# arpg/Kangaroo

Hardware: AMD Instinct MI355X
Metric: kinectfusion_frames_per_sec_640x480_to_512cubed_tsdf (higher is better)
Workload: dtype f32

## Files before the change

### include/kfx_debug.h

```cpp
#ifndef KFX_DEBUG_H
#define KFX_DEBUG_H

#include "kfx.h"

#ifdef __cplusplus
extern "C" {
#endif

int kfx_debug_rmw(const kfx_volume* vol, int variant, kfx_stream stream);

int kfx_debug_div_uniform_check(float b, unsigned long long* d_out, kfx_stream stream);

int kfx_debug_div_core_check(unsigned seed, int per_divisor, unsigned long long* d_out, kfx_stream stream);
int kfx_debug_sqrt_core_check(unsigned long long* d_out, kfx_stream stream);
int kfx_debug_wave_xor_check(unsigned seed, unsigned long long* d_out, kfx_stream stream);

int kfx_debug_summary_export(kfx_sdf_summary* s, float tol, float vref, int fine_shift, void* R_out, void* C_out, int dims_out[12],
                             kfx_stream stream);

int kfx_debug_summary_conditional_builds(kfx_sdf_summary* s, int out[2], kfx_stream stream);

int kfx_debug_summary_top_levels(kfx_sdf_summary* s, int fine_shift, void* top_out, int dims_out[12], unsigned long long* launches_out,
                                 kfx_stream stream);

int kfx_debug_fuse_keep(const kfx_sdf_summary* s, int out[3], unsigned char* kept, int n_rows);

#ifdef __cplusplus
}
#endif
#endif
```

### kangaroo_amd/csrc/debug.hip

```cpp
#include "kfx_device.h"
#include "sampling.h"
#include "../../include/kfx_debug.h"

namespace kfx {

__global__ __launch_bounds__(256) void k_rmw_linear(float4* __restrict__ base, size_t n4)
{
    const size_t stride = (size_t)gridDim.x * blockDim.x;
    for (size_t i = (size_t)blockIdx.x * blockDim.x + threadIdx.x; i < n4; i += stride) {
        float4 c = base[i];
        c.y += 1.0f;
        c.w += 1.0f;
        base[i] = c;
    }
}

template <int ZC>
__global__ __launch_bounds__(256) void k_rmw_brick(unsigned char* vptr, size_t pitch, size_t img_pitch, int X, int Y, int Z)
{
    const int tid = threadIdx.x, lane = tid & 63, wv = tid >> 6;
    const int x0 = (blockIdx.x * 32 + (lane & 31)) * 2;
    const int y = blockIdx.y * 8 + wv * 2 + (lane >> 5);
    const int zbeg = blockIdx.z * ZC, zend = min(zbeg + ZC, Z);
    if (x0 >= X || y >= Y) return;
    unsigned char* cell = vptr + (size_t)zbeg * img_pitch + (size_t)y * pitch + (size_t)x0 * 8;
    for (int z = zbeg; z < zend; ++z, cell += img_pitch) {
        float4 c = *reinterpret_cast<const float4*>(cell);
        c.y += 1.0f;
        c.w += 1.0f;
        *reinterpret_cast<float4*>(cell) = c;
    }
}

template <int ZC>
__global__ __launch_bounds__(256) void k_rmw_rows(unsigned char* vptr, size_t pitch, size_t img_pitch, int X, int Y, int Z)
{
    const int lane = threadIdx.x & 63, wv = threadIdx.x >> 6;
    const int x0 = (blockIdx.x * 64 + lane) * 2;
    const int y = blockIdx.y * 4 + wv;
    const int zbeg = blockIdx.z * ZC, zend = min(zbeg + ZC, Z);
    if (x0 >= X || y >= Y) return;
    unsigned char* cell = vptr + (size_t)zbeg * img_pitch + (size_t)y * pitch + (size_t)x0 * 8;
    for (int z = zbeg; z < zend; ++z, cell += img_pitch) {
        float4 c = *reinterpret_cast<const float4*>(cell);
        c.y += 1.0f;
        c.w += 1.0f;
        *reinterpret_cast<float4*>(cell) = c;
    }
}

__global__ __launch_bounds__(256) void k_rmw_column(unsigned char* vptr, size_t pitch, size_t img_pitch, int X, int Y, int Z)
{
    const int lane = threadIdx.x & 63, wv = threadIdx.x >> 6;
    const int x0 = (blockIdx.x * 64 + lane) * 2;
    const int y = blockIdx.y * 4 + wv;
    if (x0 >= X || y >= Y) return;
    unsigned char* cell = vptr + (size_t)y * pitch + (size_t)x0 * 8;
    for (int z = 0; z < Z; ++z, cell += img_pitch) {
        float4 c = *reinterpret_cast<const float4*>(cell);
        c.y += 1.0f;
        c.w += 1.0f;
        *reinterpret_cast<float4*>(cell) = c;
    }
}

typedef float v4f_dbg __attribute__((ext_vector_type(4)));
template <int WX, int WY, int ZC, bool NT>
__global__ __launch_bounds__(256) void k_rmw_gen(unsigned char* vptr, size_t pitch, size_t img_pitch, int X, int Y, int Z)
{
    const int lane = threadIdx.x & 63, wv = threadIdx.x >> 6;
    const int x0 = ((blockIdx.x * WX + (wv % WX)) * 64 + lane) * 2;
    const int y = blockIdx.y * WY + (wv / WX);
    const int zbeg = blockIdx.z * ZC, zend = min(zbeg + ZC, Z);
    if (x0 >= X || y >= Y) return;
    unsigned char* cell = vptr + (size_t)zbeg * img_pitch + (size_t)y * pitch + (size_t)x0 * 8;
    for (int z = zbeg; z < zend; ++z, cell += img_pitch) {
        v4f_dbg c;
        if constexpr (NT) c = __builtin_nontemporal_load(reinterpret_cast<const v4f_dbg*>(cell));
        else c = *reinterpret_cast<const v4f_dbg*>(cell);
        c.y += 1.0f;
        c.w += 1.0f;
        if constexpr (NT) __builtin_nontemporal_store(c, reinterpret_cast<v4f_dbg*>(cell));
        else *reinterpret_cast<v4f_dbg*>(cell) = c;
// ... 154 lines not shown
    GEN(12, 1, 4, 16, false)
    GEN(13, 1, 4, 16, true)
    GEN(14, 4, 1, 16, true)
    GEN(15, 1, 4, 1, false)
    GEN(16, 1, 4, 64, false)
    GEN(17, 4, 1, 4, false)
    GEN(18, 2, 2, 16, true)
#undef GEN
    default: return set_error(KFX_E_RANGE, "kfx_debug_rmw: variant");
    }
    return check_launch("kfx_debug_rmw");
}

static int last_published(const kfx_sdf_summary* s)
{
    if (!s->h_skippable || !s->builds) return -2;
    const uint64_t v = __atomic_load_n(s->h_skippable + summary_ring_index(s->builds - 1), __ATOMIC_ACQUIRE);
    return summary_ring_slot_stamp(v) == summary_ring_stamp(s->builds - 1) ? summary_ring_slot_count(v) : -1;
}

extern "C" int kfx_debug_summary_export(kfx_sdf_summary* s, float tol, float vref, int fine_shift, void* R_out, void* C_out, int dims_out[12],
                                        kfx_stream stream)
{
    if (!s || !dims_out) return set_error(KFX_E_NULL, "kfx_debug_summary_export: null argument");
    if (fine_shift < 3 || fine_shift > 5) return set_error(KFX_E_RANGE, "kfx_debug_summary_export: fine_shift in [3, 5]");
    ClassView cv;
    summary_class_layout(s, fine_shift, cv);
    dims_out[0] = s->nbx; dims_out[1] = s->nby; dims_out[2] = s->nbz;
    dims_out[3] = cv.fine.first; dims_out[4] = cv.fine.rw; dims_out[5] = cv.fine.ny;
    dims_out[6] = cv.coarse.first; dims_out[7] = cv.coarse.rw; dims_out[8] = cv.coarse.ny;
    dims_out[9] = cv.words; dims_out[10] = s->n_coarse; dims_out[11] = last_published(s);
    const size_t n = (size_t)s->nbx * s->nby * s->nbz;
    hipStream_t st = (hipStream_t)stream;
    if (R_out && hipMemcpyAsync(R_out, s->R, n * sizeof(float4), hipMemcpyDeviceToDevice, st) != hipSuccess) return set_error(KFX_E_RANGE, "kfx_debug_summary_export: copy");
    if (C_out) {
        if (int e = summary_classes_prepare(s, tol, vref, fine_shift, st)) return e;
        if (hipMemcpyAsync(C_out, s->C, (size_t)cv.words * sizeof(unsigned), hipMemcpyDeviceToDevice, st) != hipSuccess || hipStreamSynchronize(st) != hipSuccess)
            return set_error(KFX_E_RANGE, "kfx_debug_summary_export: copy");
        dims_out[11] = last_published(s);
    }
    return 0;
}

extern "C" int kfx_debug_summary_conditional_builds(kfx_sdf_summary* s, int out[2], kfx_stream stream)
{
    if (!s || !out) return set_error(KFX_E_NULL, "kfx_debug_summary_conditional_builds: null argument");
    hipStream_t st = (hipStream_t)stream;
    if (hipMemcpyAsync(out, s->d_count + 3, 2 * sizeof(int), hipMemcpyDeviceToHost, st) != hipSuccess || hipStreamSynchronize(st) != hipSuccess)
        return set_error(KFX_E_RANGE, "kfx_debug_summary_conditional_builds: copy");
    return 0;
}

extern "C" int kfx_debug_summary_top_levels(kfx_sdf_summary* s, int fine_shift, void* top_out, int dims_out[12], unsigned long long* launches_out, kfx_stream stream)
{
    if (!s || !dims_out) return set_error(KFX_E_NULL, "kfx_debug_summary_top_levels: null argument");
    if (fine_shift < 3 || fine_shift > 5) return set_error(KFX_E_RANGE, "kfx_debug_summary_top_levels: fine_shift in [3, 5]");
    ClassView cv;
    summary_class_layout(s, fine_shift, cv);
    cv.nx5 = ceil_div(s->w, 32); cv.nz5 = ceil_div(s->d, 32);
    ClassLevel l6, l7;
    int w6, w7;
    summary_top_layout(cv, l6, l7, w6, w7);
    const int nx6 = (cv.nx5 + 1) >> 1, nz6 = (cv.nz5 + 1) >> 1;
    dims_out[0] = l6.first - cv.words; dims_out[1] = l6.rw; dims_out[2] = l6.ny; dims_out[3] = nx6; dims_out[4] = nz6; dims_out[5] = w6;
    dims_out[6] = l7.first - cv.words; dims_out[7] = l7.rw; dims_out[8] = l7.ny; dims_out[9] = (nx6 + 1) >> 1; dims_out[10] = (nz6 + 1) >> 1; dims_out[11] = w7;
    if (launches_out) *launches_out = s->launches;
    if (top_out) {
        if (s->c_shift != fine_shift) return set_error(KFX_E_RANGE, "kfx_debug_summary_top_levels: the tables held were built for another fine level");
        hipStream_t st = (hipStream_t)stream;
        if (hipMemcpyAsync(top_out, s->C + cv.words, (size_t)(w6 + w7) * sizeof(unsigned), hipMemcpyDeviceToDevice, st) != hipSuccess || hipStreamSynchronize(st) != hipSuccess)
            return set_error(KFX_E_RANGE, "kfx_debug_summary_top_levels: copy");
    }
    return 0;
}

extern "C" int kfx_debug_fuse_keep(const kfx_sdf_summary* s, int out[3], unsigned char* kept, int n_rows)
{
    if (!s || !out) return set_error(KFX_E_NULL, "kfx_debug_fuse_keep: null argument");
    out[0] = s->keep_stride; out[1] = s->keep_row0; out[2] = s->keep_rows;
    for (int r = 0; kept && r < n_rows; ++r)
        kept[r] = (r >= s->keep_row0 && r < s->keep_row0 + s->keep_rows && keep_row(r, s->keep_stride)) ? 1 : 0;
    return 0;
}
```

### kangaroo_amd/csrc/frame.hip

```cpp
#include <cmath>
#include <cstdlib>
#include <new>

#include "kfx_device.h"
#include "frame_host.h"
#include "sensor_host.h"
#include "shift_host.h"

struct kfx_frame {
    kfx_frame_config cfg;
    kfx_sdf_summary* summary;
    int track;
    long long frames;
    kfx::EventRing ring;
    unsigned mask;
    kfx_image texels;
    kfx_depth_input* input;
};

using namespace kfx;

extern "C" int kfx_frame_create(kfx_frame** out, const kfx_frame_config* cfg)
{
    if (!out || !cfg) return set_error(KFX_E_NULL, "kfx_frame_create: null argument");
    *out = nullptr;
    if (!cfg->vol.ptr) return set_error(KFX_E_NULL, "kfx_frame_create: null volume");
    if (int e = check_frame_views(cfg->raw, cfg->filtered, cfg->vbo, cfg->normals, cfg->ray_depth, cfg->ray_norm, cfg->ray_img, "kfx_frame_create")) return e;
    if (cfg->timing_slots < 0 || cfg->timing_slots > (1 << 20)) return set_error(KFX_E_RANGE, "kfx_frame_create: timing_slots");
    kfx_frame* f = new (std::nothrow) kfx_frame;
    if (!f) return set_error(KFX_E_RANGE, "kfx_frame_create: out of memory");
    f->cfg = *cfg;
    f->summary = nullptr;
    f->track = 0;
    f->frames = 0;
    f->mask = KFX_FRAME_EVENTS_ALL;
    f->input = nullptr;
    f->texels = texel_image_alloc(cfg->filtered.w, cfg->filtered.h);
    if (int e = ring_create(f->ring, 4, cfg->timing_slots, -1, "kfx_frame_create")) {
        texel_image_free(f->texels);
        delete f;
        return e;
    }
    *out = f;
    return 0;
}

extern "C" int kfx_frame_destroy(kfx_frame* f)
{
    if (!f) return 0;
    if (f->summary) kfx_sdf_summary_destroy(f->summary);
    ring_destroy(f->ring);
    texel_image_free(f->texels);
    delete f;
    return 0;
}

extern "C" int kfx_frame_set_timing(kfx_frame* f, unsigned mask)
{
    if (!f) return set_error(KFX_E_NULL, "kfx_frame_set_timing: null frame");
    if (mask > KFX_FRAME_EVENTS_ALL) return set_error(KFX_E_RANGE, "kfx_frame_set_timing: mask");
    f->mask = mask;
    return 0;
}

extern "C" int kfx_frame_get_track(const kfx_frame* f) { return f ? f->track : set_error(KFX_E_NULL, "kfx_frame_get_track: null frame"); }
extern "C" kfx_sdf_summary* kfx_frame_summary(kfx_frame* f) { return f ? f->summary : nullptr; }
extern "C" long long kfx_frame_count(const kfx_frame* f) { return f ? f->frames : 0; }

kfx_volume* kfx::frame_volume(kfx_frame* f) { return &f->cfg.vol; }
kfx_sdf_summary* kfx::frame_tracked_summary(kfx_frame* f) { return f->track ? f->summary : nullptr; }

extern "C" int kfx_frame_set_track(kfx_frame* f, int on, kfx_stream stream)
{
    if (!f) return set_error(KFX_E_NULL, "kfx_frame_set_track: null frame");
    if (!on) {
        f->track = 0;
        return 0;
    }
    if (!f->summary)
        if (int e = kfx_sdf_summary_create(&f->summary, &f->cfg.vol)) return e;
    if (!f->track)
        if (int e = kfx_sdf_summary_rebuild(f->summary, stream)) return e;
    f->track = 1;
    return 0;
}

extern "C" int kfx_frame_set_input(kfx_frame* f, kfx_depth_input* in)
{
    if (!f) return set_error(KFX_E_NULL, "kfx_frame_set_input: null frame");
    if (in && !depth_input_matches(in, f->cfg.filtered.w, f->cfg.filtered.h)) return set_error(KFX_E_SHAPE, "kfx_frame_set_input: the ring's image size differs from the frame's");
    f->input = in;
    return 0;
}

extern "C" int kfx_frame_reset(kfx_frame* f, kfx_stream stream)
{
    if (!f) return set_error(KFX_E_NULL, "kfx_frame_reset: null frame");
    const float nan = __builtin_nanf("");
    if (f->track) return kfx_sdf_reset_tracked(&f->cfg.vol, f->summary, nan, stream);
    return kfx_sdf_reset(&f->cfg.vol, nan, stream);
}

extern "C" int kfx_frame_step(kfx_frame* f, const kfx_image* raw, const float T_wc[12], const float* T_cw, unsigned parts, kfx_stream stream)
{
    if (!f || !T_wc) return set_error(KFX_E_NULL, "kfx_frame_step: null argument");
    if (parts == 0) parts = KFX_FRAME_PREPROCESS | KFX_FRAME_FUSE | KFX_FRAME_RAYCAST;
    const kfx_frame_config& c = f->cfg;
    const kfx_image* src = raw ? raw : &c.raw;
    float inv[12];
    if (!T_cw) {
        se3_inverse(T_wc, inv);
        T_cw = inv;
    }
    kfx_depth_input* const sensor = (!raw && (parts & KFX_FRAME_PREPROCESS)) ? f->input : nullptr;
    if (sensor)
        if (int e0 = depth_input_wait(sensor, stream)) return e0;
    ring_begin(f->ring, f->frames, f->mask);
    int e = 0;
    const auto record = [&](int k) {
        const hipError_t he = ring_record(f->ring, f->frames, k, (hipStream_t)stream);
        if (he != hipSuccess && !e) e = set_error((int)he, "kfx_frame_step: hipEventRecord");
    };
    record(0);
    const kfx_image* tex = ((parts & KFX_FRAME_PREPROCESS) && (parts & KFX_FRAME_FUSE) && f->texels.ptr) ? &f->texels : nullptr;
    if (!e && (parts & KFX_FRAME_PREPROCESS)) {
        if (sensor) e = depth_input_consume(sensor, &c.filtered, &c.raw, c.bilateral_gs, c.bilateral_gr, c.bilateral_size, c.bilateral_minval, stream);
        else e = kfx_bilateral_f32(&c.filtered, src, c.bilateral_gs, c.bilateral_gr, c.bilateral_size, c.bilateral_minval, 1, stream);
        if (!e) e = depth_to_vbo_normals_texels(&c.vbo, &c.normals, &c.filtered, c.K, 1.0f, tex, stream);
    }
    record(1);
    if (!e && (parts & KFX_FRAME_FUSE))
        e = sdf_fuse_texels(&c.vol, f->track ? f->summary : nullptr, &c.filtered, &c.normals, tex, T_cw, c.K, c.trunc_dist, c.max_w, c.mincostheta, c.fuse_flags, stream);
    record(2);
    if (!e && (parts & KFX_FRAME_RAYCAST)) {
        if (f->track) e = kfx_raycast_sdf_tracked(&c.ray_depth, &c.ray_norm, &c.ray_img, &c.vol, f->summary, T_wc, c.K, c.near, c.far, c.trunc_dist, 1, stream);
        else e = kfx_raycast_sdf(&c.ray_depth, &c.ray_norm, &c.ray_img, &c.vol, T_wc, c.K, c.near, c.far, c.trunc_dist, 1, stream);
    }
    record(3);
    f->frames += 1;
    return e;
}

static void frame_spans(const EventRing& r, long long fr, float* o, hipError_t& he)
{
    o[0] = ring_span(r, fr, 0, 1, he);
    o[1] = ring_span(r, fr, 1, 2, he);
    o[2] = ring_span(r, fr, 2, 3, he);
    o[3] = ring_span(r, fr, 0, 3, he);
    o[4] = ring_period(r, fr, he);
}

extern "C" int kfx_frame_timings(kfx_frame* f, long long first_frame, int n_frames, float* ms)
{
    if (!f || !ms) return set_error(KFX_E_NULL, "kfx_frame_timings: null argument");
    return ring_timings(f->ring, f->frames, first_frame, n_frames, KFX_FRAME_TIMING_FIELDS, ms, frame_spans, "kfx_frame_timings");
}
```

### kangaroo_amd/csrc/frame_host.h

```cpp
#pragma once

#include <new>

#include "kfx_device.h"
#include "host_args.h"

namespace kfx {

inline int check_frame_views(const kfx_image& raw, const kfx_image& filtered, const kfx_image& vbo, const kfx_image& normals, const kfx_image& ray_depth,
                             const kfx_image& ray_norm, const kfx_image& ray_img, const char* what)
{
    const struct { const kfx_image* im; size_t elem; } views[7] = {{&raw, 4}, {&filtered, 4}, {&vbo, 16}, {&normals, 16}, {&ray_depth, 4}, {&ray_norm, 16}, {&ray_img, 4}};
    for (const auto& v : views) {
        if (!v.im->ptr) return fail_rule(what, KFX_E_SHAPE, "image views");
        if (int e = check_image(v.im, v.elem, 1, 1, what)) return e;
    }
    if (filtered.w != raw.w || filtered.h != raw.h || vbo.w != raw.w || vbo.h != raw.h || normals.w != raw.w || normals.h != raw.h)
        return fail_rule(what, KFX_E_SHAPE, "the preprocess images differ in size");
    return 0;
}

inline void se3_inverse(const float T_wc[12], float out[12])
{
    for (int i = 0; i < 3; ++i) {
        double t = 0.0;
        for (int j = 0; j < 3; ++j) {
            out[i * 4 + j] = T_wc[j * 4 + i];
            t += (double)T_wc[j * 4 + i] * (double)T_wc[j * 4 + 3];
        }
        out[i * 4 + 3] = (float)-t;
    }
}

inline kfx_image texel_image_alloc(size_t w, size_t h)
{
    const TexLayout tl = tex_layout(w, h);
    void* buf = nullptr;
    if (tl.tpitch < (1u << 24) && hipMalloc(&buf, tl.bytes) == hipSuccess) return kfx_image{tl.tpitch, buf, w, h};
    (void)hipGetLastError();
    return kfx_image{0, nullptr, 0, 0};
}
inline void texel_image_free(kfx_image& t)
{
    if (t.ptr) { (void)hipFree(t.ptr); (void)hipGetLastError(); }
    t = kfx_image{0, nullptr, 0, 0};
}

struct EventRing {
    int n = 0, slots = 0;
    int side = -1;
    hipEvent_t* ev = nullptr;
    long long* frame = nullptr;
    unsigned char* want = nullptr;
    unsigned char* mask = nullptr;
};

inline void ring_destroy(EventRing& r)
{
    if (r.ev)
        for (int i = 0; i < r.slots * r.n; ++i) if (r.ev[i]) (void)hipEventDestroy(r.ev[i]);
    delete[] r.ev; delete[] r.frame; delete[] r.want; delete[] r.mask;
    r = EventRing{};
}

inline int ring_create(EventRing& r, int n, int slots, int side, const char* what)
{
    r = EventRing{};
    if (!slots) return 0;
    r.n = n; r.slots = slots; r.side = side;
    r.ev = new (std::nothrow) hipEvent_t[(size_t)slots * n]();
    r.frame = new (std::nothrow) long long[slots];
    r.want = new (std::nothrow) unsigned char[slots]();
    r.mask = new (std::nothrow) unsigned char[slots]();
    int e = (r.ev && r.frame && r.want && r.mask) ? 0 : fail_rule(what, KFX_E_RANGE, "out of memory");
    for (int i = 0; !e && i < slots; ++i) r.frame[i] = -1;
    for (int i = 0; !e && i < slots * n; ++i) {
        const hipError_t he = hipEventCreate(&r.ev[i]);
        if (he != hipSuccess) { (void)hipGetLastError(); r.ev[i] = nullptr; e = fail_rule(what, (int)he, "hipEventCreate"); }
    }
    if (e) ring_destroy(r);
    return e;
}

inline void ring_begin(EventRing& r, long long frame, unsigned mask)
{
    if (!r.slots) return;
    const int slot = (int)(frame % r.slots);
    r.frame[slot] = mask ? frame : -1;
    r.want[slot] = (unsigned char)mask;
    r.mask[slot] = 0;
}

inline hipError_t ring_record(EventRing& r, long long frame, int k, hipStream_t stream)
{
    if (!r.slots) return hipSuccess;
    const int slot = (int)(frame % r.slots);
    if (r.frame[slot] != frame || !(r.want[slot] & (1u << k))) return hipSuccess;
    const hipError_t he = hipEventRecord(r.ev[(size_t)slot * r.n + k], stream);
    if (he == hipSuccess) r.mask[slot] |= (unsigned char)(1u << k);
    else (void)hipGetLastError();
    return he;
}

inline unsigned ring_recorded(const EventRing& r, long long frame)
{
    return frame >= 0 && r.frame[frame % r.slots] == frame ? (unsigned)r.mask[frame % r.slots] : 0u;
}
inline hipEvent_t ring_event(const EventRing& r, long long frame, int k) { return r.ev[(size_t)(frame % r.slots) * r.n + k]; }
inline int first_event(unsigned m) { return m ? __builtin_ctz(m) : -1; }
inline int last_event(unsigned m) { return m ? 31 - __builtin_clz(m) : -1; }

inline hipError_t ring_wait(const EventRing& r, long long first, long long last)
{
    hipEvent_t wait_for = nullptr;
    const int b = first_event(ring_recorded(r, last));
    if (b >= 0 && (ring_recorded(r, last + 1) & (1u << b))) wait_for = ring_event(r, last + 1, b);
    for (long long fr = last; !wait_for && fr >= first; --fr)
        if (ring_recorded(r, fr)) wait_for = ring_event(r, fr, last_event(ring_recorded(r, fr)));
    hipError_t he = wait_for ? hipEventSynchronize(wait_for) : hipSuccess;
    for (long long fr = last; r.side >= 0 && he == hipSuccess && fr >= first; --fr)
        if (ring_recorded(r, fr) & (1u << r.side)) he = hipEventSynchronize(ring_event(r, fr, r.side));
    return he;
}
// ... 39 lines not shown
```

### kangaroo_amd/csrc/fuse.hip

```cpp
#include <cmath>
#include <cstring>

#include <sys/syscall.h>
#include <unistd.h>

#include <hip/hip_fp16.h>

#include <type_traits>

#include "kfx_device.h"
#include "../../include/kfx_slab_color.h"
#include "host_args.h"

#ifndef KFX_FUSE_STAGE_DMA
#define KFX_FUSE_STAGE_DMA 1
#endif

namespace kfx {

constexpr int FUSE_ZC = 16;
constexpr int FUSE_ROWS = 4;
constexpr int TB_X = 64, TB_Y = 8;

struct FuseParams {
    unsigned char* vptr;
    size_t vpitch, vimg_pitch;
    int X, Y, Z;
    int zoff;
    float w1, h1, d1;
    V3 bmin, size;
    Pose T;
    Intr K;
    ImgView depth;
    ImgView norm;
    float dwb, dhb;
    float trunc, max_w, mincos;
    unsigned dpitch, npitch;
    int exact_shared;
    int z_rev, keep_stride, keep_row0;
    float4* sum_R;
    int sum_nbx, sum_nby;
    int sum_bx0, sum_by0, sum_bz0;
    int sum_w, sum_h, sum_d;
    float sum_lo_ok, sum_hi_ok;
    int* sum_dirty;
    int zoff_local;
    int xcd_swizzle;
    int fuse_cull;
    const unsigned char* tex;
    unsigned tpitch;
    const float* bmax;
    unsigned bw8;
    float inv_w1, inv_h1;
    int pos_div;
};

__device__ __forceinline__ float voxel_pos(float bmin, float size, int i, float n1, float inv_n1, int pos_div)
{
    const float a = size * (float)i;
    return bmin + (pos_div ? div_uniform(a, n1, inv_n1) : a / n1);
}

__device__ __forceinline__ float slice_z(const FuseParams& p, int z) { return p.bmin.z + p.size.z * (float)(z + p.zoff) / p.d1; }

__device__ __forceinline__ int xcd_rotated_brick(const FuseParams& p, int bzi)
{
    return p.xcd_swizzle ? (int)((blockIdx.x + (bzi >> (p.xcd_swizzle - 1))) % gridDim.x) : (int)blockIdx.x;
}

struct TileRect {
    int x0, y0, w, h;
    __device__ __forceinline__ bool fits(int cap) const { return w > 1 && h > 1 && w * h <= cap; }
};
__device__ __forceinline__ TileRect tile_rect(float lo_u, float hi_u, float lo_v, float hi_v, int img_w, int img_h)
{
    const float fx0 = fmaxf(floorf(lo_u) - 1.f, 0.f), fx1 = fminf(floorf(hi_u) + 2.f, (float)(img_w - 1));
    const float fy0 = fmaxf(floorf(lo_v) - 1.f, 0.f), fy1 = fminf(floorf(hi_v) + 2.f, (float)(img_h - 1));
    TileRect r;
    r.x0 = (int)fx0; r.y0 = (int)fy0;
    r.w = (int)fx1 - r.x0 + 1; r.h = (int)fy1 - r.y0 + 1;
    return r;
}
__device__ __forceinline__ bool misses_band(float lo_u, float hi_u, float lo_v, float hi_v, float wb, float hb)
{
    return hi_u < 2.0f || !(lo_u < wb) || hi_v < 2.0f || !(lo_v < hb);
}

__device__ __forceinline__ float far_depth(float dmax) { return dmax + fabsf(dmax) * 1e-5f; }
__device__ __forceinline__ bool brick_occluded(float dmax, float zmin, const FuseParams& p)
{
    return far_depth(dmax) - zmin < -(p.trunc / p.mincos) * 1.001f;
}

struct Obs {
    float val, w;
    bool ok;
};

struct Corners { float4 c00, c01, c10, c11; };
__device__ __forceinline__ Corners tile_corners(const float4* t, int tw)
{
    Corners c;
    c.c00 = t[0]; c.c01 = t[1]; c.c10 = t[tw]; c.c11 = t[tw + 1];
    return c;
}
struct CornersDx { float4 c00, d0, c10, d1; };
__device__ __forceinline__ CornersDx tile_corners_dx(const float4* t, int tw)
{
    return CornersDx{t[0], t[1], t[2 * tw], t[2 * tw + 1]};
}

typedef float v4f __attribute__((ext_vector_type(4)));

__device__ __forceinline__ float lerp_f(float a, float b, float t) { return __builtin_fmaf(t, b - a, a); }

template <bool FAST>
struct CamXY {
    float ax, ay, az;
    __device__ __forceinline__ void init(const FuseParams& p, float px, float py)
    {
        if constexpr (FAST) {
            ax = __builtin_fmaf(p.T.m[0], px, __builtin_fmaf(p.T.m[1], py, p.T.m[3]));
            ay = __builtin_fmaf(p.T.m[4], px, __builtin_fmaf(p.T.m[5], py, p.T.m[7]));
            az = __builtin_fmaf(p.T.m[8], px, __builtin_fmaf(p.T.m[9], py, p.T.m[11]));
        } else {
            ax = p.T.m[0] * px + p.T.m[1] * py;
            ay = p.T.m[4] * px + p.T.m[5] * py;
            az = p.T.m[8] * px + p.T.m[9] * py;
        }
    }
    __device__ __forceinline__ V3 at(const FuseParams& p, float pz) const
    {
        if constexpr (FAST)
            return v3(__builtin_fmaf(p.T.m[2], pz, ax), __builtin_fmaf(p.T.m[6], pz, ay), __builtin_fmaf(p.T.m[10], pz, az));
        else
            return v3(ax + p.T.m[2] * pz + p.T.m[3], ay + p.T.m[6] * pz + p.T.m[7], az + p.T.m[10] * pz + p.T.m[11]);
    }
};

template <bool FAST>
__device__ __forceinline__ void project(const FuseParams& p, const V3 Pc, float& pu, float& pv, float& iz)
{
    if constexpr (FAST) {
        iz = __builtin_amdgcn_rcpf(Pc.z);
        pu = __builtin_fmaf(p.K.fu * Pc.x, iz, p.K.u0);
        pv = __builtin_fmaf(p.K.fv * Pc.y, iz, p.K.v0);
    } else {
        iz = 0.f;
        pu = p.K.u0 + p.K.fu * Pc.x / Pc.z;
        pv = p.K.v0 + p.K.fv * Pc.y / Pc.z;
    }
}

__device__ __forceinline__ bool in_bounds(const FuseParams& p, float pu, float pv)
{
    return 2.0f <= pu && pu < p.dwb && 2.0f <= pv && pv < p.dhb;
}

__device__ __forceinline__ Corners fetch_global64(const FuseParams& p, int ix, int iy)
{
    const float* dbl = row<float>(p.depth, (size_t)iy) + ix;
    const float* dtl = row<float>(p.depth, (size_t)iy + 1) + ix;
    const float4* nbl = row<float4>(p.norm, (size_t)iy) + ix;
    const float4* ntl = row<float4>(p.norm, (size_t)iy + 1) + ix;
    const float4 n00 = nbl[0], n01 = nbl[1], n10 = ntl[0], n11 = ntl[1];
    Corners c;
    c.c00 = make_float4(n00.x, n00.y, n00.z, dbl[0]);
    c.c01 = make_float4(n01.x, n01.y, n01.z, dbl[1]);
    c.c10 = make_float4(n10.x, n10.y, n10.z, dtl[0]);
    c.c11 = make_float4(n11.x, n11.y, n11.z, dtl[1]);
    return c;
}

struct __attribute__((packed, aligned(4))) P2 { float a, b; };
__device__ __forceinline__ Corners fetch_global32(const FuseParams& p, int ix, int iy)
{
    const unsigned od = __umul24((unsigned)iy, p.dpitch) + (unsigned)ix * 4u;
    const unsigned on = __umul24((unsigned)iy, p.npitch) + (unsigned)ix * 16u;
    const P2 db = *reinterpret_cast<const P2*>(p.depth.ptr + od);
    const P2 dt = *reinterpret_cast<const P2*>(p.depth.ptr + p.dpitch + od);
    const float4* nb = reinterpret_cast<const float4*>(p.norm.ptr + on);
    const float4* nt = reinterpret_cast<const float4*>(p.norm.ptr + p.npitch + on);
    const float4 n00 = nb[0], n01 = nb[1], n10 = nt[0], n11 = nt[1];
    Corners c;
    c.c00 = make_float4(n00.x, n00.y, n00.z, db.a);
    c.c01 = make_float4(n01.x, n01.y, n01.z, db.b);
    c.c10 = make_float4(n10.x, n10.y, n10.z, dt.a);
    c.c11 = make_float4(n11.x, n11.y, n11.z, dt.b);
    return c;
}

template <bool FAST>
__device__ __forceinline__ Obs finish(const FuseParams& p, const V3 Pc, float iz, float fx, float fy, const Corners& c)
{
    Obs o;
    o.ok = false;
    o.val = 0.f;
    o.w = 0.f;
    float md, costheta, w;
    if constexpr (FAST) {
        md = lerp_f(lerp_f(c.c00.w, c.c01.w, fx), lerp_f(c.c10.w, c.c11.w, fx), fy);
        const float nx = lerp_f(lerp_f(c.c00.x, c.c01.x, fx), lerp_f(c.c10.x, c.c11.x, fx), fy);
        const float ny = lerp_f(lerp_f(c.c00.y, c.c01.y, fx), lerp_f(c.c10.y, c.c11.y, fx), fy);
        const float nz = lerp_f(lerp_f(c.c00.z, c.c01.z, fx), lerp_f(c.c10.z, c.c11.z, fx), fy);
        const float dotn = __builtin_fmaf(nz, Pc.z, __builtin_fmaf(ny, Pc.y, nx * Pc.x));
        const float len2 = __builtin_fmaf(Pc.z, Pc.z, __builtin_fmaf(Pc.y, Pc.y, Pc.x * Pc.x));
        costheta = -dotn * __builtin_amdgcn_rsqf(len2);
        w = costheta * iz;
    } else {
        md = lerp(lerp(c.c00.w, c.c01.w, fx), lerp(c.c10.w, c.c11.w, fx), fy);
        V3 mdn;
        mdn.x = lerp(lerp(c.c00.x, c.c01.x, fx), lerp(c.c10.x, c.c11.x, fx), fy);
        mdn.y = lerp(lerp(c.c00.y, c.c01.y, fx), lerp(c.c10.y, c.c11.y, fx), fy);
        mdn.z = lerp(lerp(c.c00.z, c.c01.z, fx), lerp(c.c10.z, c.c11.z, fx), fy);
        costheta = dot(mdn, Pc) / -length(Pc);
        w = costheta * 1.0f / Pc.z;
    }
    const float sd = costheta * (md - Pc.z);
    o.ok = ((int)!(sd <= -p.trunc) & (int)isfinite(md) & (int)isfinite(w) & (int)(costheta > p.mincos)) != 0;
    if constexpr (FAST) o.val = __builtin_amdgcn_fmed3f(sd, -p.trunc, p.trunc);
    else o.val = clampf(sd, -p.trunc, p.trunc);
    o.w = w;
    return o;
}

__device__ __forceinline__ Obs finish_shared(const FuseParams& p, const V3 Pc, float yz, float fx, float fy, const Corners& c)
{
    Obs o;
    const float md = lerp(lerp(c.c00.w, c.c01.w, fx), lerp(c.c10.w, c.c11.w, fx), fy);
    V3 mdn;
    mdn.x = lerp(lerp(c.c00.x, c.c01.x, fx), lerp(c.c10.x, c.c11.x, fx), fy);
    mdn.y = lerp(lerp(c.c00.y, c.c01.y, fx), lerp(c.c10.y, c.c11.y, fx), fy);
    mdn.z = lerp(lerp(c.c00.z, c.c01.z, fx), lerp(c.c10.z, c.c11.z, fx), fy);
    const float nlen = -sqrt_core(dot(Pc, Pc));
    const float costheta = div_core(dot(mdn, Pc), nlen, rcp_nr(nlen));
// ... 131 lines not shown
    o.w = 0.f;
    float pu, pv, iz;
    project<FAST>(p, Pc, pu, pv, iz);
    if (in_bounds(p, pu, pv)) {
        const float fix = floorf(pu), fiy = floorf(pv);
        const Corners c = TEX ? fetch_texels(p, (int)fix, (int)fiy) : (OFF32 ? fetch_global32(p, (int)fix, (int)fiy) : fetch_global64(p, (int)fix, (int)fiy));
        o = finish<FAST>(p, Pc, iz, pu - fix, pv - fiy, c);
    }
    return o;
}

template <int VEC, bool FAST, bool OFF32, typename CELL>
__global__ __launch_bounds__(256) void k_sdf_fuse(const FuseParams p)
{
    __shared__ float s_pz[FUSE_ZC];
    const int lane = threadIdx.x & 63, wv = threadIdx.x >> 6;
    const int x0 = (blockIdx.x * 64 + lane) * VEC;
    const int y = blockIdx.y * FUSE_ROWS + wv;
    const int zbeg = blockIdx.z * FUSE_ZC;
    const int zend = min(zbeg + FUSE_ZC, p.Z);
    if (threadIdx.x < FUSE_ZC)
        s_pz[threadIdx.x] = slice_z(p, zbeg + (int)threadIdx.x);
    __syncthreads();
    if (x0 >= p.X || y >= p.Y) return;

    const float py = p.bmin.y + p.size.y * (float)y / p.h1;
    CamXY<FAST> cam[VEC];
#pragma unroll
    for (int v = 0; v < VEC; ++v) cam[v].init(p, p.bmin.x + p.size.x * (float)(x0 + v) / p.w1, py);

    unsigned char* cell = p.vptr + (size_t)zbeg * p.vimg_pitch + (size_t)y * p.vpitch + (size_t)x0 * CELL::BYTES;
    for (int z = zbeg; z < zend; ++z, cell += p.vimg_pitch) {
        const float pz = s_pz[z - zbeg];
        Obs o[VEC];
#pragma unroll
        for (int v = 0; v < VEC; ++v) o[v] = observe<FAST, OFF32>(p, cam[v].at(p, pz));
        if constexpr (VEC == 2) {
            if (o[0].ok || o[1].ok) {
                float4 c = CELL::ld2(cell);
                accumulate_pair<FAST, CELL>(o[0], o[1], p.max_w, c);
                CELL::st2(cell, c);
            }
        } else {
            if (o[0].ok) {
                float2 c = CELL::ld1(cell);
                accumulate<FAST, CELL>(o[0], p.max_w, c.x, c.y);
                CELL::st1(cell, c);
            }
        }
    }
}

template <bool FAST, int ZU, typename CELL, int LX = 32, int WY = 4, int ZC = FUSE_ZC, bool TRACK = false, bool DXT = false, int NW = 4>
__global__ __launch_bounds__(64 * NW, (FAST && ZU == 2) ? 8 : (!FAST ? 6 : 1)) void k_sdf_fuse_tiled(const FuseParams p_arg, const int cap_px)
{
    static_assert(!DXT || (!FAST && !TRACK), "the difference tile belongs to the bit-exact, untracked kernels");
    FuseParams p = p_arg;
    constexpr bool PARK = !(FAST && TRACK);
    if constexpr (PARK) {
        p.T.m[2] = in_vgpr(p.T.m[2]); p.T.m[6] = in_vgpr(p.T.m[6]); p.T.m[10] = in_vgpr(p.T.m[10]);
        if constexpr (!FAST) { p.T.m[3] = in_vgpr(p.T.m[3]); p.T.m[7] = in_vgpr(p.T.m[7]); p.T.m[11] = in_vgpr(p.T.m[11]); }
        p.K.fu = in_vgpr(p.K.fu); p.K.fv = in_vgpr(p.K.fv); p.K.u0 = in_vgpr(p.K.u0); p.K.v0 = in_vgpr(p.K.v0);
    }
    constexpr int NT = 64 * NW, RW = 64 / LX, WZ = NW / WY, ZW = ZC / WZ, BY = RW * WY;
    static_assert(LX * RW == 64 && WY * WZ == NW && ZW * WZ == ZC && ZW % ZU == 0, "brick geometry");
    static_assert(NW == 4 || (NW == 8 && !TRACK), "the summary epilogue is written for four waves");
    constexpr int NG = ZW / 8, NXB = LX / 4, NZB = ZC / 8;
    static_assert(!TRACK || (BY == 8 && ZW % 8 == 0 && NG <= 2 && 8 % ZU == 0), "summary bricks are 8 x 8 x 8");
    __shared__ float s_part[TRACK ? 4 * 2 * 8 * 3 : 1];
    extern __shared__ __attribute__((aligned(16))) float4 s_tile[];
    __shared__ float s_pz[ZC];
    __shared__ float s_dmax[NW], s_cmin[NW];
    __shared__ float4 s_tz[ZC];
    const int tid = threadIdx.x, lane = tid & 63, wv = __builtin_amdgcn_readfirstlane(tid >> 6);
    const int bzi = (TRACK && p.z_rev) ? (int)(gridDim.z - 1 - blockIdx.z) : (int)blockIdx.z;
    const int bxi = xcd_rotated_brick(p, bzi);
    const int x0 = (bxi * LX + (lane & (LX - 1))) * 2;
    const int y = blockIdx.y * BY + (wv % WY) * RW + lane / LX;
    const int zbeg = bzi * ZC;
    const bool keep = TRACK && keep_row(p.keep_row0 + (int)blockIdx.y, p.keep_stride);
    const int zend = min(zbeg + ZC, p.Z);
    const int wz0 = zbeg + (wv / WY) * ZW, wz1 = min(wz0 + ZW, zend);
    const bool live = x0 < p.X && y < p.Y;
    if (tid < ZC) {
        const float pz = slice_z(p, zbeg + tid);
        s_pz[tid] = pz;
        if constexpr (!FAST) s_tz[tid] = make_float4(pz, p.T.m[2] * pz, p.T.m[6] * pz, p.T.m[10] * pz);
    }
    __syncthreads();

    const float py = voxel_pos(p.bmin.y, p.size.y, y, p.h1, p.inv_h1, p.pos_div);
    CamXY<FAST> cam[2];
#pragma unroll
    for (int v = 0; v < 2; ++v) cam[v].init(p, voxel_pos(p.bmin.x, p.size.x, x0 + v, p.w1, p.inv_w1, p.pos_div), py);

    float umin, umax, vmin, vmax, zmin, cmax = 0.f;
    bool any_bad;
    {
        const int c = lane & 7;
        const int xb0 = bxi * LX * 2, yb0 = (int)blockIdx.y * BY;
        const int xc = (c & 1) ? min(xb0 + LX * 2, p.X) - 1 : xb0;
        const int yc = (c & 2) ? min(yb0 + BY, p.Y) - 1 : yb0;
        const float pzc = s_pz[(c & 4) ? (zend - 1 - zbeg) : 0];
        CamXY<FAST> cc;
        cc.init(p, voxel_pos(p.bmin.x, p.size.x, xc, p.w1, p.inv_w1, p.pos_div), voxel_pos(p.bmin.y, p.size.y, yc, p.h1, p.inv_h1, p.pos_div));
        const V3 Pc = cc.at(p, pzc);
        float pu, pv, iz;
        project<FAST>(p, Pc, pu, pv, iz);
        const bool bad = !(Pc.z > 0.f) || !(fabsf(pu) < 1e9f) || !(fabsf(pv) < 1e9f);
        const FMin fmin2;
        const FMax fmax2;
        const auto uni = [](float x) { return __uint_as_float((unsigned)__builtin_amdgcn_readfirstlane((int)__float_as_uint(x))); };
        umin = uni(wave8_combine(pu, fmin2)); umax = uni(wave8_combine(pu, fmax2));
        vmin = uni(wave8_combine(pv, fmin2)); vmax = uni(wave8_combine(pv, fmax2));
        zmin = uni(wave8_combine(Pc.z, fmin2));
        if constexpr (!FAST) cmax = uni(wave8_combine(fmaxf(fmaxf(fabsf(Pc.x), fabsf(Pc.y)), Pc.z), fmax2));
        any_bad = __ballot(bad) != 0ull;
    }

    bool use_tile = false;
    TileRect tile = {0, 0, 0, 0};
    if (!any_bad) {
        if (misses_band(umin, umax, vmin, vmax, p.dwb, p.dhb)) return;
        tile = tile_rect(umin, umax, vmin, vmax, p.depth.w, p.depth.h);
        use_tile = tile.fits(cap_px);
        if constexpr (DXT) use_tile = use_tile && p.exact_shared && zmin >= 0x1p-20f && cmax <= 0x1p20f;
    }
    const int tx0 = tile.x0, ty0 = tile.y0, tw = tile.w, th = tile.h;
    const bool whole = !TRACK || ((bxi + 1) * LX * 2 <= p.X && ((int)blockIdx.y + 1) * BY <= p.Y);
    const bool interior = __builtin_amdgcn_readfirstlane((int)(use_tile && whole && umin >= 2.01f && umax < p.dwb - 0.01f && vmin >= 2.01f && vmax < p.dhb - 0.01f)) != 0;
    float dmax = -__builtin_inff();
    constexpr bool DMA = KFX_FUSE_STAGE_DMA && !DXT;
    if constexpr (DMA) {
        if (use_tile) {
            const unsigned lane16 = (unsigned)lane * 16u;
            const unsigned lds0 = (unsigned)(size_t)(__attribute__((address_space(3))) char*)(char*)s_tile;
            const int tail = tw & 63;
            const unsigned long long mask_tail = tail ? ((1ull << tail) - 1ull) : ~0ull;
            const int chunks = (tw + 63) >> 6;
            for (int r = wv; r < th; r += NW) {
                const unsigned char* rowp = p.tex + ((size_t)(ty0 + r) * p.tpitch + (size_t)tx0 * 16u);
                unsigned dst = lds0 + (unsigned)(r * tw) * 16u;
#pragma unroll 1
                for (int c = 0; c < chunks; ++c, rowp += 1024, dst += 1024u) {
                    const unsigned long long m = (c + 1 == chunks) ? mask_tail : ~0ull;
                    unsigned long long keep_exec;
                    unsigned keep_m0;
                    asm volatile("s_mov_b64 %0, exec\n\t"
                                 "s_mov_b32 %1, m0\n\t"
                                 "s_mov_b64 exec, %2\n\t"
                                 "s_mov_b32 m0, %3\n\t"
                                 "s_nop 0\n\t"
                                 "global_load_lds_dwordx4 %4, %5\n\t"
                                 "s_mov_b32 m0, %1\n\t"
                                 "s_mov_b64 exec, %0"
                                 : "=&s"(keep_exec), "=&s"(keep_m0)
                                 : "s"(m), "s"(dst), "v"(lane16), "s"(rowp)
                                 : "memory");
                }
            }
            {
                const int bx0 = tx0 >> 3, nbx = ((tx0 + tw - 1) >> 3) - bx0 + 1, by0 = ty0 >> 2, nb = nbx * (((ty0 + th - 1) >> 2) - by0 + 1);
                const float inv_nbx = 1.0f / (float)nbx;
                for (int i = tid; i < nb; i += NT) {
                    const int br = (int)(((float)i + 0.5f) * inv_nbx);
                    dmax = fmaxf(dmax, p.bmax[(size_t)(by0 + br) * p.bw8 + (size_t)(bx0 + i - br * nbx)]);
                }
                block_put(s_dmax, wv, dmax, FMax{});
            }
            asm volatile("s_waitcnt vmcnt(0)" ::: "memory");
        }
    }
    if (!DMA && use_tile) {
        if constexpr (FAST) {
            const int ntex = tw * th;
            const float inv_tw = 1.0f / (float)tw;
            constexpr int SU = 4;
            for (int t0 = tid; t0 < ntex; t0 += NT * SU) {
                float4 n[SU];
                float d[SU];
#pragma unroll
                for (int k = 0; k < SU; ++k) {
                    const int t = t0 + k * NT;
                    n[k] = make_float4(0.f, 0.f, 0.f, 0.f);
                    d[k] = -__builtin_inff();
                    if (t < ntex) {
                        const int r = (int)(((float)t + 0.5f) * inv_tw);
                        const int c = t - r * tw;
                        const unsigned y = (unsigned)(ty0 + r), x = (unsigned)(tx0 + c);
                        n[k] = *reinterpret_cast<const float4*>(p.norm.ptr + (__umul24(y, p.npitch) + x * 16u));
                        d[k] = *reinterpret_cast<const float*>(p.depth.ptr + (__umul24(y, p.dpitch) + x * 4u));
                    }
                }
#pragma unroll
                for (int k = 0; k < SU; ++k) {
                    const int t = t0 + k * NT;
                    if (t < ntex) {
                        s_tile[t] = make_float4(n[k].x, n[k].y, n[k].z, d[k]);
                        dmax = fmaxf(dmax, d[k]);
                    }
                }
            }
        } else {
            for (int r = wv; r < th; r += NW) {
                const float* drow = row<float>(p.depth, (size_t)(ty0 + r)) + tx0;
                const float4* nrow = row<float4>(p.norm, (size_t)(ty0 + r)) + tx0;
                for (int c = lane; c < tw; c += 64) {
                    const float4 n = nrow[c];
                    const float d = drow[c];
                    s_tile[(r * tw + c) * (DXT ? 2 : 1)] = make_float4(n.x, n.y, n.z, d);
                    dmax = fmaxf(dmax, d);
                }
            }
// ... 123 lines not shown
                const float fix = floorf(pu), fiy = floorf(pv);
                const int ix = (int)fix, iy = (int)fiy;
                const unsigned rx = (unsigned)(ix - tx0), ry = (unsigned)(iy - ty0);
                Corners c;
                if (use_tile && rx < (unsigned)(tw - 1) && ry < (unsigned)(th - 1)) {
                    c = tile_corners(s_tile + (ry * (unsigned)tw + rx), tw);
                } else {
                    c = DMA ? fetch_texels(p, ix, iy) : fetch_global32(p, ix, iy);
                }
                o = finish<FAST>(p, Pc, iz, pu - fix, pv - fiy, c);
            }
            return o;
        };

        unsigned char* cell = p.vptr + (size_t)wz0 * p.vimg_pitch + (size_t)y * p.vpitch + (size_t)x0 * CELL::BYTES;

        if constexpr (!FAST) {
            if (use_tile && p.exact_shared && zmin >= 0x1p-20f && cmax <= 0x1p20f) {
                const int cxmax = in_vgpr(tw - 2), cymax = in_vgpr(th - 2), tx0v = in_vgpr(tx0), ty0v = in_vgpr(ty0);
                auto observe_pair = [&](auto interior_c, int z, Obs (&o)[2]) -> bool {
                    constexpr bool INTERIOR = decltype(interior_c)::value;
                    const float4 tz = s_tz[z - zbeg];
                    bool stray = false;
    #pragma unroll
                    for (int v = 0; v < 2; ++v) {
                        const V3 Pc = v3(cam[v].ax + tz.y + p.T.m[3], cam[v].ay + tz.z + p.T.m[7], cam[v].az + tz.w + p.T.m[11]);
                        const float yz = rcp_nr(Pc.z);
                        const float pu = p.K.u0 + div_core(p.K.fu * Pc.x, Pc.z, yz);
                        const float pv = p.K.v0 + div_core(p.K.fv * Pc.y, Pc.z, yz);
                        const float fix = floorf(pu), fiy = floorf(pv);
                        const int rx = (int)fix - tx0v, ry = (int)fiy - ty0v;
                        const auto sample = [&](int at) {
                            if constexpr (DXT) return finish_shared(p, Pc, yz, pu - fix, pv - fiy, tile_corners_dx(s_tile + 2 * at, tw));
                            else return finish_shared(p, Pc, yz, pu - fix, pv - fiy, tile_corners(s_tile + at, tw));
                        };
                        if constexpr (INTERIOR) {
                            o[v] = sample(ry * tw + rx);
                        } else {
                            const bool inb = upd && in_bounds(p, pu, pv), inside = cell_inside(rx, ry, cxmax, cymax);
                            o[v] = sample(cell_clamped(rx, ry, cxmax, cymax, tw));
                            stray |= gate_sample(o[v], inb, inside);
                        }
                    }
                    if constexpr (!INTERIOR) {
                        if (__builtin_expect(__ballot(stray) != 0ull, 0)) {
                            o[0] = observe<false, true, DMA>(p, cam[0].at(p, tz.x));
                            o[1] = observe<false, true, DMA>(p, cam[1].at(p, tz.x));
                            o[0].ok = o[0].ok && upd; o[1].ok = o[1].ok && upd;
                        }
                    }
                    return ((int)o[0].ok | (int)o[1].ok) != 0;
                };
                auto shared_loop = [&](auto interior_c) {
                for (int z = wz0; z < wz1; z += ZU, cell += (size_t)ZU * p.vimg_pitch) {
                    next_group(z);
                    Obs o[ZU][2];
                    bool any[ZU];
    #pragma unroll
                    for (int k = 0; k < ZU; ++k) {
                        any[k] = false;
                        if (z + k < wz1) {
                            any[k] = observe_pair(interior_c, z + k, o[k]);
                            note_pair(o[k][0].ok, o[k][1].ok);
                        }
                    }
                    float4 c[ZU];
                    load_cells(c, any, cell);
    #pragma unroll
                    for (int k = 0; k < ZU; ++k)
                        if (any[k]) {
                            accumulate_pair<false, CELL>(o[k][0], o[k][1], p.max_w, c[k]);
                            CELL::st2(cell + (size_t)k * p.vimg_pitch, c[k]);
                            note_vals(c[k]);
                        }
                }
                };
                if (interior) shared_loop(std::true_type{});
                else shared_loop(std::false_type{});
                flush();
                return;
            }
        }
        if (use_tile) {
            const int cxmax = PARK ? in_vgpr(tw - 2) : tw - 2, cymax = PARK ? in_vgpr(th - 2) : th - 2, tx0v = PARK ? in_vgpr(tx0) : tx0,
                      ty0v = PARK ? in_vgpr(ty0) : ty0;
            auto tiled_loop = [&](auto interior_c) {
            constexpr bool INTERIOR = decltype(interior_c)::value;
            for (int z = wz0; z < wz1; z += ZU, cell += (size_t)ZU * p.vimg_pitch) {
                next_group(z);
                Obs o[ZU][2];
                bool any[ZU];
                bool stray = false;
    #pragma unroll
                for (int k = 0; k < ZU; ++k) {
                    any[k] = false;
                    if (z + k < wz1) {
                        const float pz = s_pz[z + k - zbeg];
    #pragma unroll
                        for (int v = 0; v < 2; ++v) {
                            const V3 Pc = cam[v].at(p, pz);
                            float pu, pv, iz;
                            project<FAST>(p, Pc, pu, pv, iz);
                            const float fix = floorf(pu), fiy = floorf(pv);
                            const int rx = (int)fix - tx0v, ry = (int)fiy - ty0v;
                            if constexpr (INTERIOR) {
                                o[k][v] = finish<FAST>(p, Pc, iz, pu - fix, pv - fiy, tile_corners(s_tile + (ry * tw + rx), tw));
                            } else {
                                const bool inb = upd && in_bounds(p, pu, pv), inside = cell_inside(rx, ry, cxmax, cymax);
                                o[k][v] = finish<FAST>(p, Pc, iz, pu - fix, pv - fiy, tile_corners(s_tile + cell_clamped(rx, ry, cxmax, cymax, tw), tw));
                                stray |= gate_sample(o[k][v], inb, inside);
                            }
                        }
                        any[k] = ((int)o[k][0].ok | (int)o[k][1].ok) != 0;
                    }
                }
                if constexpr (!INTERIOR) {
                if (__builtin_expect(__ballot(stray) != 0ull, 0)) {
    #pragma unroll
                    for (int k = 0; k < ZU; ++k)
                        if (z + k < wz1) {
                            const float pz = s_pz[z + k - zbeg];
                            o[k][0] = observe<FAST, true, DMA>(p, cam[0].at(p, pz));
                            o[k][1] = observe<FAST, true, DMA>(p, cam[1].at(p, pz));
                            o[k][0].ok = o[k][0].ok && upd; o[k][1].ok = o[k][1].ok && upd;
                            any[k] = o[k][0].ok || o[k][1].ok;
                        }
                }
                }
    #pragma unroll
                for (int k = 0; k < ZU; ++k)
                    if (z + k < wz1) note_pair(o[k][0].ok, o[k][1].ok);
                float4 c[ZU];
                load_cells(c, any, cell);
    #pragma unroll
                for (int k = 0; k < ZU; ++k)
                    if (any[k]) {
                        if (o[k][0].ok) accumulate<FAST, CELL>(o[k][0], p.max_w, c[k].x, c[k].y);
                        if (o[k][1].ok) accumulate<FAST, CELL>(o[k][1], p.max_w, c[k].z, c[k].w);
                        CELL::st2(cell + (size_t)k * p.vimg_pitch, c[k]);
                        note_vals(c[k]);
                    }
            }
            };
            if (interior) tiled_loop(std::true_type{});
            else tiled_loop(std::false_type{});
            flush();
            return;
        }
        for (int z = wz0; z < wz1; z += ZU, cell += (size_t)ZU * p.vimg_pitch) {
            next_group(z);
            Obs o[ZU][2];
            bool any[ZU];
    #pragma unroll
            for (int k = 0; k < ZU; ++k) {
                any[k] = false;
                if (z + k < wz1) {
                    const float pz = s_pz[z + k - zbeg];
                    o[k][0] = observe_tile(0, pz);
                    o[k][1] = observe_tile(1, pz);
                    o[k][0].ok = o[k][0].ok && upd; o[k][1].ok = o[k][1].ok && upd;
                    any[k] = o[k][0].ok || o[k][1].ok;
                    note_pair(o[k][0].ok, o[k][1].ok);
                }
            }
            float4 c[ZU];
            load_cells(c, any, cell);
    #pragma unroll
// ... 408 lines not shown
        }
        block_put(s_dmax, wv, dmax, FMax{});
    }
    __syncthreads();
    if (use_tile && p.mincos > 0.f && p.trunc > 0.f && brick_occluded(block_get<4>(s_dmax, FMax{}), zmin, p)) return;
    if constexpr (!TRACK) {
        if (!live) return;
    }
    const bool upd = !TRACK || live;
    ColorTrack trk;
    trk.reset(0);

    unsigned char* cell = p.vptr + (size_t)zbeg * p.vimg_pitch + (size_t)y * p.vpitch + (size_t)x0 * 8;
    unsigned char* ccell = q.cptr + (size_t)zbeg * q.cimg_pitch + (size_t)y * q.cpitch + (size_t)x0 * 4;
    const int cxmax = tw - 2, cymax = th - 2, gxmax = cw - 2, gymax = chh - 2;
    for (int z = zbeg; z < zend; ++z, cell += p.vimg_pitch, ccell += q.cimg_pitch) {
        if constexpr (TRACK) trk.next_group(s_part, wv, lane, zend - zbeg, z - zbeg);
        const float pz = s_pz[z - zbeg];
        Obs o[2];
        float grey[2];
        bool stray = !use_tile;
        if (use_tile) {
#pragma unroll
            for (int v = 0; v < 2; ++v) {
                const V3 Pc = cam[v].at(p, pz), Pi = ccam[v].at(q, pz);
                float pu, pv, iz, qu, qv;
                project<FAST>(p, Pc, pu, pv, iz);
                project_color<FAST>(q, Pi, qu, qv);
                const bool inb = upd && in_bounds(p, pu, pv) && in_bounds_color(q, qu, qv);
                const float fix = floorf(pu), fiy = floorf(pv), gix = floorf(qu), giy = floorf(qv);
                const int rx = (int)fix - tx0, ry = (int)fiy - ty0, gx = (int)gix - cx0, gy = (int)giy - cy0;
                const bool inside = cell_inside(rx, ry, cxmax, cymax) && cell_inside(gx, gy, gxmax, gymax);
                o[v] = finish<FAST>(p, Pc, iz, pu - fix, pv - fiy, tile_corners(s_tile + cell_clamped(rx, ry, cxmax, cymax, tw), tw));
                stray |= gate_sample(o[v], inb, inside);
                const unsigned* g = s_rgb + cell_clamped(gx, gy, gxmax, gymax, cw);
                const Rgb4 texels{g[0], g[1], g[cw], g[cw + 1]};
                if constexpr (FAST) {
                    grey[v] = grey_bilinear<true>(texels, qu - gix, qv - giy);
                } else {
                    grey[v] = 0.f;
                    if (o[v].ok) grey[v] = grey_bilinear<false>(texels, qu - gix, qv - giy);
                }
            }
        }
        if (__builtin_expect(__ballot(stray) != 0ull, 0)) {
#pragma unroll
            for (int v = 0; v < 2; ++v) {
                o[v] = observe_color_global<FAST>(p, q, cam[v].at(p, pz), ccam[v].at(q, pz), grey[v]);
                o[v].ok = o[v].ok && upd;
            }
        }
        if constexpr (TRACK) trk.note_pair(o[0].ok, o[1].ok);
        if (o[0].ok || o[1].ok) {
            float4 c = CellF32::ld2(cell);
            const v2f k = __builtin_nontemporal_load(reinterpret_cast<const v2f*>(ccell));
            float k0 = k.x, k1 = k.y;
            if (o[0].ok) k0 = color_mean<FAST>(o[0].w, grey[0], k0, c.y);
            if (o[1].ok) k1 = color_mean<FAST>(o[1].w, grey[1], k1, c.w);
            accumulate_pair<FAST, CellF32>(o[0], o[1], p.max_w, c);
            CellF32::st2(cell, c);
            v2f kk;
            kk.x = k0; kk.y = k1;
            __builtin_nontemporal_store(kk, reinterpret_cast<v2f*>(ccell));
            if constexpr (TRACK) trk.note_vals(c);
        }
    }
    if constexpr (TRACK) {
        trk.flush(s_part, wv, lane, zend - zbeg);
        __syncthreads();
        color_track_epilogue(p, s_part, tid, bxi, zbeg);
    }
}

__global__ __launch_bounds__(256) void k_fill_f32(float* __restrict__ base, size_t n, float v)
{
    for (size_t i = (size_t)blockIdx.x * 256 + threadIdx.x; i < n; i += (size_t)gridDim.x * 256) base[i] = v;
}

}

using namespace kfx;

__global__ __launch_bounds__(256) void k_pack_texels(const ImgView depth, const ImgView norm, unsigned char* __restrict__ tex, const size_t tpitch,
                                                     float* __restrict__ bmax, const unsigned bw8)
{
    __shared__ float s_max[PIX_H][8];
    int u, v, lane, wv;
    pixel_xy(u, v, lane, wv);
    float d = -__builtin_inff();
    if (u < depth.w && v < depth.h) {
        d = row<float>(depth, (size_t)v)[u];
        texel_put(tex, tpitch, u, v, row<float4>(norm, (size_t)v)[u], d);
    }
    texel_block_max(bmax, bw8, lane, wv, d, s_max);
}

struct TexScratch {
    static constexpr int N = 4;
    struct Entry { void* buf; size_t bytes; hipStream_t stream; int device; unsigned long used; };
    Entry e[N] = {};
    unsigned long tick = 0;
    bool main_thread = false;
    ~TexScratch()
    {
        if (main_thread) return;
        for (Entry& x : e)
            if (x.buf) { (void)hipFree(x.buf); (void)hipGetLastError(); }
    }
    void* get(size_t bytes, hipStream_t stream)
    {
        int dev = 0;
        if (hipGetDevice(&dev) != hipSuccess) { (void)hipGetLastError(); return nullptr; }
        Entry* hit = nullptr;
        Entry* lru = &e[0];
        for (Entry& x : e) {
            if (x.buf && x.stream == stream && x.device == dev) { hit = &x; break; }
            if (!x.buf) { if (lru->buf) lru = &x; } else if (lru->buf && x.used < lru->used) lru = &x;
        }
        if (!hit) {
            hit = lru;
            if (hit->buf) {
                (void)hipFree(hit->buf); (void)hipGetLastError();
                hit->buf = nullptr; hit->bytes = 0;
            }
            hit->stream = stream; hit->device = dev;
        }
        if (hit->bytes < bytes) {
            if (hit->buf) { (void)hipFree(hit->buf); (void)hipGetLastError(); hit->buf = nullptr; hit->bytes = 0; }
            if (hipMalloc(&hit->buf, bytes) != hipSuccess) { (void)hipGetLastError(); hit->buf = nullptr; return nullptr; }
            hit->bytes = bytes;
        }
        hit->used = ++tick;
        return hit->buf;
    }
};
static void* tex_scratch(size_t bytes, hipStream_t stream)
{
    thread_local TexScratch pool;
    static const long main_tid = (long)getpid();
    pool.main_thread = (long)syscall(SYS_gettid) == main_tid;
    return pool.get(bytes, stream);
}

static VolView vol_view(const kfx_volume* vol)
{
    VolView v;
    v.ptr = (unsigned char*)vol->ptr;
    v.pitch = vol->pitch;
    v.img_pitch = vol->img_pitch;
    v.w = (int)vol->w;
    v.h = (int)vol->h;
    v.d = (int)vol->d;
    v.bmin = V3{vol->boxmin[0], vol->boxmin[1], vol->boxmin[2]};
    v.bmax = V3{vol->boxmax[0], vol->boxmax[1], vol->boxmax[2]};
    return v;
}

static bool pos_div_verified(int axis, float size, int dim)
{
    struct Memo { float size; int dim; bool ok; };
    static thread_local Memo memo[2] = {{0.0f, 0, false}, {0.0f, 0, false}};
    Memo& m = memo[axis];
    if (m.dim == dim && memcmp(&m.size, &size, sizeof(float)) == 0) return m.ok;
    const float n1 = (float)(dim - 1), inv = 1.0f / n1;
    bool ok = div_uniform_safe_host(size) && div_uniform_safe_host(size * n1);
    for (int i = 0; ok && i < dim; ++i) {
        const float a = size * (float)i;
        const float q0 = a * inv;
        const float q = fmaf(fmaf(-n1, q0, a), inv, q0), d = a / n1;
// ... 21 lines not shown
    p.Z = full ? (int)vol->d : (int)(vol->d / 8) * 8;
    if (!full && (flags & KFX_FUSE_SLAB_EXTENT) && slab) {
        const size_t zlim = (slab->full_d / 8) * 8;
        const size_t z_end = slab->z_offset + vol->d < zlim ? slab->z_offset + vol->d : zlim;
        p.Z = z_end > slab->z_offset ? (int)(z_end - slab->z_offset) : 0;
    }
    p.w1 = (float)(vol->w - 1);
    p.h1 = (float)(vol->h - 1);
    p.d1 = (float)(vol->d - 1);
    p.bmin = V3{vol->boxmin[0], vol->boxmin[1], vol->boxmin[2]};
    p.size = V3{vol->boxmax[0] - vol->boxmin[0], vol->boxmax[1] - vol->boxmin[1], vol->boxmax[2] - vol->boxmin[2]};
    if (slab) {
        if (slab->full_d < 2 || slab->z_offset + vol->d > slab->full_d) return set_error(KFX_E_SHAPE, "SdfFuse: slab outside the full volume");
        p.d1 = (float)(slab->full_d - 1);
        p.zoff = (int)slab->z_offset;
        p.bmin.z = slab->full_zmin;
        p.size.z = slab->full_zmax - slab->full_zmin;
    }
    for (int i = 0; i < 12; ++i) p.T.m[i] = T_cw[i];
    p.K = Intr{K[0], K[1], K[2], K[3]};
    p.depth = ImgView{(const unsigned char*)depth->ptr, depth->pitch, (int)depth->w, (int)depth->h};
    p.norm = ImgView{(const unsigned char*)norm->ptr, norm->pitch, (int)norm->w, (int)norm->h};
    p.dwb = (float)depth->w - 2.0f;
    p.dhb = (float)depth->h - 2.0f;
    p.trunc = trunc_dist;
    p.max_w = max_w;
    p.mincos = mincostheta;
    *small_images = depth->pitch * depth->h < (1ull << 31) && norm->pitch * norm->h < (1ull << 31) &&
                    depth->pitch < (1u << 24) && norm->pitch < (1u << 24) && depth->h < (1u << 24);
    p.dpitch = *small_images ? (unsigned)depth->pitch : 0u;
    p.npitch = *small_images ? (unsigned)norm->pitch : 0u;
    p.inv_w1 = 1.0f / p.w1;
    p.inv_h1 = 1.0f / p.h1;
    static const int pos_div_env = env_int("KFX_FUSE_POS_DIV", 1);
    p.pos_div = (pos_div_env && vol->w >= 2 && vol->h >= 2 && pos_div_verified(0, p.size.x, (int)vol->w) && pos_div_verified(1, p.size.y, (int)vol->h)) ? 1 : 0;
    static const int swizzle_env = env_int("KFX_FUSE_XCD_SWIZZLE", 1, 0, 8);
    p.xcd_swizzle = swizzle_env;
    static const int cull_env = env_int("KFX_FUSE_CULL", 1);
    p.fuse_cull = cull_env;
    static const int shared_env = env_int("KFX_FUSE_EXACT_SHARED", 1);
    const float afu = fabsf(p.K.fu), afv = fabsf(p.K.fv);
    p.exact_shared = shared_env && afu >= 0x1p-20f && afu <= 0x1p20f && afv >= 0x1p-20f && afv <= 0x1p20f &&
                     mincostheta >= 0x1p-20f && mincostheta < __builtin_inff() && trunc_dist > 0.f && trunc_dist < __builtin_inff();
    return 0;
}

static float px_per_voxel(const FuseParams& p, const Pose& T, const Intr& K, int z0, int z1)
{
    const float cx = p.bmin.x + 0.5f * p.size.x, cy = p.bmin.y + 0.5f * p.size.y;
    const float cz = p.bmin.z + p.size.z * (0.5f * (float)(z0 + z1 - 1) + (float)p.zoff) / p.d1;
    const float Zc = T.m[8] * cx + T.m[9] * cy + T.m[10] * cz + T.m[11];
    if (!(Zc > 0.f)) return 0.f;
    const float voxel = fmaxf(p.size.x / p.w1, p.size.y / p.h1);
    return fmaxf(fabsf(K.fu), fabsf(K.fv)) * voxel / Zc;
}

static int tile_cap(const FuseParams& p, const Pose& T, const Intr& K, int z0, int z1, bool small_ok = false)
{
    const float r = px_per_voxel(p, T, K, z0, z1);
    static const float r_small = env_float("KFX_FUSE_R_SMALL", 0.85f);
    if (small_ok && !(r > r_small)) return 1216;
    if (!(r > 1.3f)) return 1536;
    const float want = 1536.f * (r / 1.05f) * (r / 1.05f);
    const int c = want >= 3072.f ? 3072 : ((int)want + 511) / 512 * 512;
    return c < 1536 ? 1536 : c;
}

struct TilePlan { int small_brick, cap, dxt; };
static bool operator==(const TilePlan& a, const TilePlan& b) { return a.cap == b.cap && a.small_brick == b.small_brick && a.dxt == b.dxt; }
static TilePlan tile_plan(const FuseParams& p, const Pose& T, const Intr& K, int z0, int z1, int brick_env, bool fast)
{
    const float r = px_per_voxel(p, T, K, z0, z1);
    const int small_brick = brick_env < 0 ? (r > 1.3f ? 1 : 0) : (brick_env != 0);
    static const float r_dxt = 0.01f * (float)env_int("KFX_FUSE_DXT", 64);
    if (!small_brick && !fast && r_dxt > 0.f && r > 0.f && !(r > r_dxt)) return TilePlan{0, 768, 1};
    if (!small_brick) return TilePlan{0, tile_cap(p, T, K, z0, z1, fast), 0};
    const float want = 0.75f * (r * 41.f + 5.f) * (r * 14.7f + 5.f);
    const int caps[] = {1216, 1600, 1984, 2496, 3328};
    for (int c : caps)
        if (want <= (float)c) return TilePlan{small_brick, c, 0};
    return TilePlan{small_brick, 3328, 0};
}

static int fuse_tiled_env()
{
    static const int tiled = env_int("KFX_FUSE_TILED", 1);
    return tiled;
}

constexpr int FUSE_ZSTEP = 64;
template <typename PLAN, typename F>
static int merged_range_end(int z0, int Z, PLAN& plan, F plan_of)
{
    int z1 = z0 + FUSE_ZSTEP < Z ? z0 + FUSE_ZSTEP : Z;
    plan = plan_of(z0, z1);
    while (z1 < Z) {
        const int z2 = z1 + FUSE_ZSTEP < Z ? z1 + FUSE_ZSTEP : Z;
        if (!(plan_of(z1, z2) == plan)) break;
        z1 = z2;
    }
    return z1;
}

static FuseParams z_range(const FuseParams& p, int z0, int z1)
{
    FuseParams q = p;
    q.vptr = p.vptr + (size_t)z0 * p.vimg_pitch;
    q.zoff = p.zoff + z0;
    q.zoff_local = z0;
    q.Z = z1 - z0;
    return q;
}

struct TiledKernel {
    void (*fn)(FuseParams, int);
    int bx, by, bz, threads;
    dim3 grid(const FuseParams& q) const { return dim3(ceil_div(q.X, bx), ceil_div(q.Y, by), ceil_div(q.Z, bz)); }
};
template <bool FAST, int ZU, typename CELL, int LX, int WY, bool TRACK = false, bool DXT = false, int NW = 4>
static TiledKernel tiled_kernel()
{
    return TiledKernel{k_sdf_fuse_tiled<FAST, ZU, CELL, LX, WY, FUSE_ZC, TRACK, DXT, NW>, LX * 2, 64 / LX * WY, FUSE_ZC, 64 * NW};
}
template <typename CELL, int LX, int WY>
static TiledKernel tiled_kernel_for(bool fast, int zu, bool track, bool dxt, bool nw8)
{
    if (track) return fast ? tiled_kernel<true, 2, CELL, LX, WY, true>() : tiled_kernel<false, 1, CELL, LX, WY, true>();
    if constexpr (LX == 16) {
        if (nw8) return tiled_kernel<true, 2, CELL, LX, WY, false, false, 8>();
    }
    if (fast) return zu == 4 ? tiled_kernel<true, 4, CELL, LX, WY>() : zu == 2 ? tiled_kernel<true, 2, CELL, LX, WY>() : tiled_kernel<true, 1, CELL, LX, WY>();
    if constexpr (LX == 32) {
        if (zu == 2) return tiled_kernel<false, 2, CELL, LX, WY>();
        if (dxt) return tiled_kernel<false, 1, CELL, LX, WY, false, true>();
    }
    return tiled_kernel<false, 1, CELL, LX, WY>();
}
template <typename CELL>
static TiledKernel tiled_kernel_for(bool fast, int zu, bool small_brick, bool track, bool dxt, bool nw8)
{
    return small_brick ? tiled_kernel_for<CELL, 16, 2>(fast, zu, track, dxt, nw8) : tiled_kernel_for<CELL, 32, 4>(fast, zu, track, dxt, false);
}

template <int VEC, typename CELL>
static void launch_generic(const FuseParams& p, bool fast, bool small_images, hipStream_t s)
{
    const dim3 grid(ceil_div(p.X, 64 * VEC), ceil_div(p.Y, FUSE_ROWS), ceil_div(p.Z, FUSE_ZC));
    if (fast && small_images) hipLaunchKernelGGL((k_sdf_fuse<VEC, true, true, CELL>), grid, dim3(256), 0, s, p);
    else if (fast) hipLaunchKernelGGL((k_sdf_fuse<VEC, true, false, CELL>), grid, dim3(256), 0, s, p);
    else if (small_images) hipLaunchKernelGGL((k_sdf_fuse<VEC, false, true, CELL>), grid, dim3(256), 0, s, p);
    else hipLaunchKernelGGL((k_sdf_fuse<VEC, false, false, CELL>), grid, dim3(256), 0, s, p);
}

static int summary_hookup(FuseParams& p, bool* track, kfx_sdf_summary* summary, const kfx_volume* vol, bool empty, bool can_track, kfx_stream stream)
{
    *track = false;
    if (!summary) return 0;
    int ox, oy, oz;
    if (int e = summary_view_offset(summary, vol, &ox, &oy, &oz)) return e;
    *track = (ox % 8 == 0) && (oy % 8 == 0) && (oz % 8 == 0);
    p.sum_R = summary->R;
    p.sum_nbx = summary->nbx; p.sum_nby = summary->nby;
    p.sum_bx0 = ox / 8; p.sum_by0 = oy / 8; p.sum_bz0 = oz / 8;
    p.sum_w = summary->w; p.sum_h = summary->h; p.sum_d = summary->d;
    p.sum_lo_ok = summary->c_lo_ok; p.sum_hi_ok = summary->c_hi_ok;
    p.sum_dirty = summary->d_dirty;
    if (empty) return 0;
    if (!(*track && can_track)) {
        if (int e = kfx_sdf_summary_invalidate(summary, stream)) return e;
        *track = false;
    }
    if (!summary->c_dirty) summary->c_dirty = 1;
    return 0;
}

template <typename CELL>
static int fuse_launch(const kfx_volume* vol, const kfx_image* depth, const kfx_image* norm, const float T_cw[12],
                       const float K[4], float trunc_dist, float max_w, float mincostheta, unsigned flags, kfx_stream stream,
                       const kfx_slab* slab = nullptr, kfx_sdf_summary* summary = nullptr, const kfx_image* texels = nullptr)
{
    FuseParams p;
    bool small_images = false;
    if (int e = fuse_params(p, &small_images, vol, depth, norm, T_cw, K, trunc_dist, max_w, mincostheta, flags, CELL::BYTES, slab)) return e;
    if (summary && summary->cell_bytes != CELL::BYTES)
        return set_error(KFX_E_SHAPE, "SdfFuse(tracked): the summary was created for the other cell type (kfx_sdf_summary_create / _create_h)");
    const bool empty = p.X == 0 || p.Y == 0 || p.Z == 0;
    const bool vec2 = (p.X % 2 == 0) && ((((uintptr_t)vol->ptr | vol->pitch | vol->img_pitch) & (2 * CELL::BYTES - 1)) == 0);
    const int tiled = fuse_tiled_env();
    bool track = false;
    if (int e = summary_hookup(p, &track, summary, vol, empty, tiled && vec2 && small_images, stream)) return e;
    if (empty) return 0;
    const bool fast = math_mode() == KFX_MATH_FAST;
    hipStream_t s = (hipStream_t)stream;
    static const int cap_env = [] { const int v = env_int("KFX_FUSE_CAP", 0); return v <= 0 ? 0 : (v < 64 ? 64 : (v > 3968 ? 3968 : v)); }();
    if (tiled && vec2 && small_images) {
        static const int zu_env = env_int("KFX_FUSE_ZU", 0);
        static const int brick_env = env_int("KFX_FUSE_BRICK", -1);
        auto plan_for = [&](int z0, int z1) -> TilePlan {
            TilePlan t = tile_plan(p, p.T, p.K, z0, z1, brick_env, fast);
            if (track || CELL::BYTES != 8) {
                if (t.dxt) t = TilePlan{0, tile_cap(p, p.T, p.K, z0, z1, fast), 0};
            }
            if (cap_env) { t.cap = cap_env; t.dxt = 0; }
            return t;
        };
        bool all_dxt = true;
        for (int z = 0; z < p.Z; z += FUSE_ZSTEP) all_dxt = all_dxt && plan_for(z, z + FUSE_ZSTEP < p.Z ? z + FUSE_ZSTEP : p.Z).dxt != 0;
        auto plan_of = [&](int za, int zb) -> TilePlan {
            TilePlan t = plan_for(za, zb);
            if (t.dxt && !all_dxt) { t = TilePlan{0, tile_cap(p, p.T, p.K, za, zb, fast), 0}; if (cap_env) t.cap = cap_env; }
            return t;
        };
        static const int keep_mb = env_int("KFX_FUSE_KEEP_MB", 256);
        const int rev = (track && keep_mb > 0) ? (int)(summary->sweeps++ & 1u) : 0;
        int keep_stride = 0;
        if (track && keep_mb > 0 && fast && CELL::BYTES == 8) {
            const size_t vol_bytes = summary->img_pitch * (size_t)summary->d, budget = (size_t)keep_mb << 20;
            keep_stride = (int)((vol_bytes + budget - 1) / budget);
            if (keep_stride < 1) keep_stride = 1;
        }
        if (track) { summary->keep_stride = keep_stride; summary->keep_row0 = p.sum_by0; summary->keep_rows = ceil_div(p.Y, TB_Y); }
        struct Range { int z0, z1; TilePlan plan; };
        Range ranges[64];
        int n_ranges = 0;
        for (int z0 = 0; z0 < p.Z;) {
            TilePlan plan;
            const int z1 = merged_range_end(z0, p.Z, plan, plan_of);
            if (n_ranges == 64) { ranges[63].z1 = p.Z; break; }
            ranges[n_ranges++] = Range{z0, z1, plan};
            z0 = z1;
        }
        bool any_plain = false;
        for (int ri = 0; ri < n_ranges; ++ri) any_plain = any_plain || !ranges[ri].plan.dxt;
        if (KFX_FUSE_STAGE_DMA && any_plain) {
            const TexLayout tl = tex_layout(depth->w, depth->h);
            if (texels && texels->ptr && texels->w == depth->w && texels->h == depth->h && texels->pitch == tl.tpitch && !((uintptr_t)texels->ptr & 15)) {
                p.tex = (const unsigned char*)texels->ptr;
            } else {
                void* buf = tex_scratch(tl.bytes, s);
                if (!buf) return set_error((int)hipErrorOutOfMemory, "SdfFuse: no device memory for the packed texel image");
                hipLaunchKernelGGL(k_pack_texels, pixel_grid((int)depth->w, (int)depth->h), dim3(256), 0, s, p.depth, p.norm,
                                   (unsigned char*)buf, tl.tpitch, reinterpret_cast<float*>((unsigned char*)buf + tl.bmax_off), tl.bw8);
                p.tex = (const unsigned char*)buf;
            }
            p.tpitch = (unsigned)tl.tpitch;
            p.bmax = reinterpret_cast<const float*>(p.tex + tl.bmax_off);
            p.bw8 = tl.bw8;
        }
        static const int nw8_from = env_int("KFX_FUSE_NW8", 2048);
        for (int ri = 0; ri < n_ranges; ++ri) {
            const Range& rg = ranges[rev ? n_ranges - 1 - ri : ri];
            const TilePlan plan = rg.plan;
            const int cap_px = plan.cap;
            FuseParams q = z_range(p, rg.z0, rg.z1);
            q.z_rev = rev;
            q.keep_stride = keep_stride; q.keep_row0 = p.sum_by0;
            const size_t lds = (size_t)cap_px * sizeof(float4) * (plan.dxt ? 2 : 1);
            const int zu = zu_env ? zu_env : (fast ? (cap_px > 2560 ? 4 : 2) : 1);
            const bool nw8 = fast && nw8_from > 0 && cap_px > nw8_from;
            const TiledKernel k = tiled_kernel_for<CELL>(fast, zu, plan.small_brick != 0, track, plan.dxt != 0, nw8);
            hipLaunchKernelGGL(k.fn, k.grid(q), dim3(k.threads), lds, s, q, cap_px);
        }
    } else if (vec2) {
        launch_generic<2, CELL>(p, fast, small_images, s);
    } else {
        launch_generic<1, CELL>(p, fast, small_images, s);
    }
    return check_launch("kfx_sdf_fuse");
}

extern "C" int kfx_sdf_fuse(const kfx_volume* vol, const kfx_image* depth, const kfx_image* norm,
                            const float T_cw[12], const float K[4], float trunc_dist, float max_w,
                            float mincostheta, unsigned flags, kfx_stream stream)
{
    return fuse_launch<CellF32>(vol, depth, norm, T_cw, K, trunc_dist, max_w, mincostheta, flags, stream);
}

int kfx::sdf_fuse_texels(const kfx_volume* vol, kfx_sdf_summary* summary, const kfx_image* depth, const kfx_image* norm, const kfx_image* texels,
                         const float T_cw[12], const float K[4], float trunc_dist, float max_w, float mincostheta, unsigned flags, kfx_stream stream)
{
    return fuse_launch<CellF32>(vol, depth, norm, T_cw, K, trunc_dist, max_w, mincostheta, flags, stream, nullptr, summary, texels);
}

int kfx::sdf_fuse_slab_texels(const kfx_volume* vol, const kfx_slab* slab, const kfx_image* depth, const kfx_image* norm, const kfx_image* texels,
                              const float T_cw[12], const float K[4], float trunc_dist, float max_w, float mincostheta, unsigned flags, kfx_stream stream)
{
    if (!slab) return set_error(KFX_E_NULL, "kfx_sdf_fuse_slab: null slab");
    return fuse_launch<CellF32>(vol, depth, norm, T_cw, K, trunc_dist, max_w, mincostheta, flags, stream, slab, nullptr, texels);
}

extern "C" int kfx_sdf_fuse_tracked(const kfx_volume* vol, kfx_sdf_summary* summary, const kfx_image* depth, const kfx_image* norm,
                                    const float T_cw[12], const float K[4], float trunc_dist, float max_w, float mincostheta,
                                    unsigned flags, kfx_stream stream)
{
    if (!summary) return set_error(KFX_E_NULL, "kfx_sdf_fuse_tracked: null summary");
    return fuse_launch<CellF32>(vol, depth, norm, T_cw, K, trunc_dist, max_w, mincostheta, flags, stream, nullptr, summary);
}

extern "C" int kfx_sdf_fuse_slab(const kfx_volume* vol, const kfx_slab* slab, const kfx_image* depth, const kfx_image* norm,
                                 const float T_cw[12], const float K[4], float trunc_dist, float max_w,
                                 float mincostheta, unsigned flags, kfx_stream stream)
{
    if (!slab) return set_error(KFX_E_NULL, "kfx_sdf_fuse_slab: null slab");
    return fuse_launch<CellF32>(vol, depth, norm, T_cw, K, trunc_dist, max_w, mincostheta, flags, stream, slab);
}

extern "C" int kfx_sdf_fuse_slab_h(const kfx_volume* vol, const kfx_slab* slab, const kfx_image* depth, const kfx_image* norm,
                                   const float T_cw[12], const float K[4], float trunc_dist, float max_w,
                                   float mincostheta, unsigned flags, kfx_stream stream)
{
    if (!slab) return set_error(KFX_E_NULL, "kfx_sdf_fuse_slab_h: null slab");
    return fuse_launch<CellF16>(vol, depth, norm, T_cw, K, trunc_dist, max_w, mincostheta, flags, stream, slab);
}

extern "C" int kfx_sdf_fuse_h(const kfx_volume* vol, const kfx_image* depth, const kfx_image* norm,
                              const float T_cw[12], const float K[4], float trunc_dist, float max_w,
                              float mincostheta, unsigned flags, kfx_stream stream)
{
    return fuse_launch<CellF16>(vol, depth, norm, T_cw, K, trunc_dist, max_w, mincostheta, flags, stream);
}

extern "C" int kfx_sdf_fuse_tracked_h(const kfx_volume* vol, kfx_sdf_summary* summary, const kfx_image* depth, const kfx_image* norm,
                                      const float T_cw[12], const float K[4], float trunc_dist, float max_w, float mincostheta,
                                      unsigned flags, kfx_stream stream)
{
    if (!summary) return set_error(KFX_E_NULL, "kfx_sdf_fuse_tracked_h: null summary");
    return fuse_launch<CellF16>(vol, depth, norm, T_cw, K, trunc_dist, max_w, mincostheta, flags, stream, nullptr, summary);
}

extern "C" int kfx_sdf_fuse_count(const kfx_volume* vol, const kfx_image* depth, const kfx_image* norm,
                                  const float T_cw[12], const float K[4], float trunc_dist, float mincostheta,
                                  unsigned flags, unsigned long long* d_count, kfx_stream stream)
{
    if (!d_count) return set_error(KFX_E_NULL, "kfx_sdf_fuse_count: null counter");
    FuseParams p;
    bool small_images = false;
    if (int e = fuse_params(p, &small_images, vol, depth, norm, T_cw, K, trunc_dist, 0.f, mincostheta, flags, 8, nullptr)) return e;
    if (p.X == 0 || p.Y == 0 || p.Z == 0) return 0;
    const int bx = ceil_div(p.X, 64), by = ceil_div(p.Y, FUSE_ROWS), bz = ceil_div(p.Z, FUSE_ZC);
    const long long total = (long long)bx * by * bz;
    if (total > 0x7fffffffLL) return set_error(KFX_E_RANGE, "kfx_sdf_fuse_count: volume too large");
    dim3 grid((unsigned)(total < 4096 ? total : 4096));
    if (math_mode() == KFX_MATH_FAST) hipLaunchKernelGGL(k_sdf_fuse_count<true>, grid, dim3(256), 0, (hipStream_t)stream, p, bx, by, bz, d_count);
    else hipLaunchKernelGGL(k_sdf_fuse_count<false>, grid, dim3(256), 0, (hipStream_t)stream, p, bx, by, bz, d_count);
    return check_launch("kfx_sdf_fuse_count");
}

extern "C" int kfx_sdf_reset(const kfx_volume* vol, float trunc_dist, kfx_stream stream)
{
    if (int e = check_volume(vol, 8, 1, VOLUME_MAX_DIM, "SdfReset")) return e;
    const size_t span_bytes = (vol->d - 1) * vol->img_pitch + (vol->h - 1) * vol->pitch + vol->w * 8;
    const size_t n = span_bytes / 8;
    const int blocks = (int)std::min<size_t>((n / 2 + 255) / 256 + 1, 256 * 32);
    hipStream_t s = (hipStream_t)stream;
    if (((uintptr_t)vol->ptr & 15) == 0)
        hipLaunchKernelGGL(k_fill_sdf, dim3((unsigned)((n / 2 + 1023) / 1024 + 1)), dim3(256), 0, s, (float2*)vol->ptr, n, trunc_dist, 0.0f);
    else
        hipLaunchKernelGGL(k_fill_sdf_unaligned, dim3(blocks), dim3(256), 0, s, (float2*)vol->ptr, n, trunc_dist, 0.0f);
    return check_launch("kfx_sdf_reset");
}

template <typename CELL>
static int sphere_launch(const kfx_volume* vol, const float center[3], float r, kfx_stream stream, const char* what)
{
// ... 128 lines not shown
```

### kangaroo_amd/csrc/kfx_device.h

```cpp
#pragma once

#include <hip/hip_runtime.h>
#include <stddef.h>
#include <stdint.h>

#include "../../include/kfx.h"
#include "../../include/kfx_extras.h"
#include "../../include/kfx_summary_h.h"
#include "../../include/kfx_color.h"
#include "summary_ring_host.h"

namespace kfx {

struct V3 { float x, y, z; };

__device__ __forceinline__ V3 v3(float x, float y, float z) { return V3{x, y, z}; }
__device__ __forceinline__ V3 operator+(V3 a, V3 b) { return V3{a.x + b.x, a.y + b.y, a.z + b.z}; }
__device__ __forceinline__ V3 operator-(V3 a, V3 b) { return V3{a.x - b.x, a.y - b.y, a.z - b.z}; }
__device__ __forceinline__ V3 operator*(V3 a, float s) { return V3{a.x * s, a.y * s, a.z * s}; }
__device__ __forceinline__ V3 div_cw(V3 a, V3 b) { return V3{a.x / b.x, a.y / b.y, a.z / b.z}; }
__device__ __forceinline__ V3 div_s(V3 a, float s) { const float inv = 1.0f / s; return a * inv; }
__device__ __forceinline__ float dot(V3 a, V3 b) { return a.x * b.x + a.y * b.y + a.z * b.z; }
__device__ __forceinline__ float length(V3 a) { return sqrtf(dot(a, a)); }
__device__ __forceinline__ float lerp(float a, float b, float t) { return a + t * (b - a); }
// ... 233 lines not shown
    unsigned long long launches;
    unsigned plain_calls;
    unsigned sweeps;
    int keep_stride, keep_row0, keep_rows;
};
namespace kfx {
struct ClassLevel {
    int shift;
    int ny;
    int rw;
    int first;
};
struct ClassView {
    const unsigned* C;
    ClassLevel fine, coarse;
    int words;
    float vref;
    float tol;
    int amb_ok;
    int ox, oy, oz;
    float eps;
    int nx5, nz5, top_n, lds_words;
    int global, top_first;
};
__device__ __forceinline__ unsigned brick_class_mask(const float lo, const float hi, const int state, const float lo_ok, const float hi_ok)
{
    const bool in_band = lo >= lo_ok && hi <= hi_ok;
    return (state == 1 ? 1u : 0u) | ((state == 0 && in_band) ? 2u : 0u) | ((state == 1 || in_band) ? 4u : 0u);
}
inline __host__ __device__ void class_level_up(const int nx, const int ny, const int nz, const int shift, const int first, ClassLevel& L, int& ux, int& uz, int& words)
{
    ux = (nx + 1) >> 1; uz = (nz + 1) >> 1;
    L.shift = shift; L.ny = (ny + 1) >> 1; L.rw = 2 * ((ux + 31) >> 5); L.first = first;
    words = (L.rw * L.ny * uz + 3) & ~3;
}
__device__ __forceinline__ void classes_level_up(unsigned* tab, const ClassLevel& src, int snx, int snz, const ClassLevel& dst, int dnx, int dnz)
{
    const int lane = threadIdx.x & 63;
    int lg = 0;
    while ((1 << lg) < dnx && lg < 6) ++lg;
    const int chunks = (dnx + 63) >> 6;
    const int px = chunks > 1 ? chunks << 6 : 1 << lg;
    const int total = px * dst.ny * dnz;
    for (int e0 = 0; e0 < total; e0 += 256) {
        const int e = e0 + (int)threadIdx.x;
        const int bx = chunks > 1 ? e % px : e & (px - 1), r = chunks > 1 ? e / px : e >> lg;
        const int by = r % dst.ny, bz = r / dst.ny;
        int cls = 0;
        if (e < total && bx < dnx) {
            bool all_free = true, all_nan = true, all_either = true;
#pragma unroll
            for (int k = 0; k < 8; ++k) {
                const int x = min(2 * bx + (k & 1), snx - 1), y = min(2 * by + ((k >> 1) & 1), src.ny - 1), z = min(2 * bz + (k >> 2), snz - 1);
                const uint2 w = *reinterpret_cast<const uint2*>(tab + src.first + (z * src.ny + y) * src.rw + ((x >> 5) << 1));
                const int c = (int)((w.x >> (x & 31)) & 1u) | (int)(((w.y >> (x & 31)) & 1u) << 1);
                all_free = all_free && c == 1;
                all_nan = all_nan && c == 2;
                all_either = all_either && c != 0;
            }
            cls = all_free ? 1 : (all_nan ? 2 : (all_either ? 3 : 0));
        }
        const unsigned long long p0 = __ballot(cls & 1), p1 = __ballot(cls & 2);
        if (e < total && (bx & 63) == 0 && (chunks > 1 || bx == 0)) {
            const int sh = chunks > 1 ? 0 : lane;
            const unsigned long long m = (chunks > 1 || lg == 6) ? ~0ull : ((1ull << (1 << lg)) - 1ull);
            const unsigned long long r0 = (p0 >> sh) & m, r1 = (p1 >> sh) & m;
            unsigned* out = tab + dst.first + (bz * dst.ny + by) * dst.rw + (bx >> 6) * 4;
            out[0] = (unsigned)r0; out[1] = (unsigned)r1;
            if ((bx >> 6) * 4 + 2 < dst.rw) { out[2] = (unsigned)(r0 >> 32); out[3] = (unsigned)(r1 >> 32); }
        }
    }
}
int summary_classes_prepare(kfx_sdf_summary* s, float tol, float vref, int fine_shift, hipStream_t stream, int global = 0);
void summary_class_layout(const kfx_sdf_summary* s, int fine_shift, ClassView& cv);
void summary_top_layout(const ClassView& cv, ClassLevel& l6, ClassLevel& l7, int& w6, int& w7);
int summary_view_offset(const kfx_sdf_summary* s, const kfx_volume* view, int* ox, int* oy, int* oz);
}

namespace kfx {
int set_error(int code, const char* what);
int check_launch(const char* what);
int hip_status(hipError_t e, const char* what);
int math_mode();
int depth_to_vbo_normals_texels(const kfx_image* vbo, const kfx_image* nrm, const kfx_image* depth, const float K[4], float scale,
                                const kfx_image* texels, kfx_stream stream);
int sdf_fuse_slab_texels(const kfx_volume* vol, const kfx_slab* slab, const kfx_image* depth, const kfx_image* norm, const kfx_image* texels,
                         const float T_cw[12], const float K[4], float trunc_dist, float max_w, float mincostheta, unsigned flags, kfx_stream stream);
int sdf_fuse_texels(const kfx_volume* vol, kfx_sdf_summary* summary, const kfx_image* depth, const kfx_image* norm, const kfx_image* texels,
                    const float T_cw[12], const float K[4], float trunc_dist, float max_w, float mincostheta, unsigned flags, kfx_stream stream);
}
```

### kangaroo_amd/csrc/preprocess.hip

```cpp

#include "kfx_device.h"
#include "host_args.h"
#include "sensor_host.h"

namespace kfx {

constexpr int BIL_MAX_R = 16;

struct BilParams {
    const unsigned char* in;
    size_t in_pitch;
    unsigned char* out;
    size_t out_pitch;
    int w, h;
    int iw, ih;
    int R;
    float gs, gr;
    float minval;
    int use_minval;
};

template <typename Ti>
__device__ __forceinline__ float load_clamped(const BilParams& p, int x, int y)
{
    x = min(max(x, 0), p.iw - 1);
    y = min(max(y, 0), p.ih - 1);
    return (float)reinterpret_cast<const Ti*>(p.in + (size_t)y * p.in_pitch)[x];
}

__device__ __forceinline__ float scale_bias(float a, float s, float offset) { return s * a + offset; }

struct AsLoaded {
    __device__ __forceinline__ float operator()(float v) const { return v; }
    __device__ __forceinline__ void keep(int, int, float) const {}
};
struct ToMetres {
    unsigned char* metres;
    size_t mpitch;
    float s, offset;
    __device__ __forceinline__ float operator()(float v) const { return scale_bias(v, s, offset); }
    __device__ __forceinline__ void keep(int x, int y, float m) const
    {
        if (metres) reinterpret_cast<float*>(metres + (size_t)y * mpitch)[x] = m;
    }
};

template <typename Ti, int TX, int TY, int PY, typename Conv>
__global__ __launch_bounds__(TX * TY) void k_bilateral(const BilParams p, const Conv conv)
{
    extern __shared__ __attribute__((aligned(16))) float lds[];
    constexpr int NT = TX * TY;
    const int R = p.R, D = 2 * R + 1;
    const int TW = TX + 2 * R, TH = TY * PY + 2 * R;
    float* tile = lds;
    float* sw = lds + TW * TH;
    const int tid = threadIdx.x;
    const int bx = blockIdx.x * TX, by = blockIdx.y * (TY * PY);

    for (int i = tid; i < TW * TH; i += NT) {
        const int ty = i / TW, tx = i - ty * TW;
        tile[i] = conv(load_clamped<Ti>(p, bx + tx - R, by + ty - R));
    }
    for (int i = tid; i < D * D; i += NT) {
        const int r = i / D - R, c = i % D - R;
        const float sd2 = (float)(r * r + c * c);
        sw[i] = __expf(-(sd2) / (2 * p.gs * p.gs));
    }
    __syncthreads();

    const int lx = tid % TX, ly0 = tid / TX;
    const int x = bx + lx;
    if (x >= p.w) return;
    const float inv2gr = 2 * p.gr * p.gr;
#pragma unroll
    for (int k = 0; k < PY; ++k) {
        const int ly = ly0 + k * TY;
        const int y = by + ly;
        if (y >= p.h) break;
        const float pc = tile[(ly + R) * TW + lx + R];
        conv.keep(x, y, pc);
        float sum = 0.f, sumw = 0.f;
        if (!p.use_minval || pc >= p.minval) {
            for (int r = 0; r < D; ++r) {
                const float* trow = tile + (ly + r) * TW + lx;
// ... 79 lines not shown
            }
    }
    reinterpret_cast<float*>(p.out + (size_t)y * p.out_pitch)[x] = sum / sumw;
}

struct GuidedParams {
    BilParams b;
    const unsigned char* guide;
    size_t gpitch;
    int gw, gh;
    float gc;
};
template <typename Tg>
__global__ __launch_bounds__(256) void k_bilateral_guided(const GuidedParams g)
{
    const BilParams& p = g.b;
    int x, y;
    pixel_xy(x, y);
    if (x >= p.w || y >= p.h) return;
    const float pv = reinterpret_cast<const float*>(p.in + (size_t)y * p.in_pitch)[x];
    const float pcv = (float)reinterpret_cast<const Tg*>(g.guide + (size_t)y * g.gpitch)[x];
    float sum = 0.f, sumw = 0.f;
    for (int r = -p.R; r <= p.R; ++r)
        for (int c = -p.R; c <= p.R; ++c) {
            const float q = load_clamped<float>(p, x + c, y + r);
            const int gx = min(max(x + c, 0), g.gw - 1), gy = min(max(y + r, 0), g.gh - 1);
            const float qc = (float)reinterpret_cast<const Tg*>(g.guide + (size_t)gy * g.gpitch)[gx];
            const float rd = pv - q, cd = pcv - qc;
            const float sd2 = (float)(r * r + c * c);
            const float rd2 = rd * rd, cd2 = cd * cd;
            const float sw = __expf(-(sd2) / (2 * p.gs * p.gs));
            const float rw = __expf(-(rd2) / (2 * p.gr * p.gr));
            const float cw = __expf(-(cd2) / (2 * g.gc * g.gc));
            const float w = sw * rw * cw;
            sumw += w;
            sum += w * q;
        }
    reinterpret_cast<float*>(p.out + (size_t)y * p.out_pitch)[x] = sumw == 0 ? pv : sum / sumw;
}

struct PixOp {
    const unsigned char* in;
    size_t in_pitch;
    unsigned char* out;
    size_t out_pitch;
    int w, h;
};
template <typename T>
__device__ __forceinline__ const T* in_row(const PixOp& p, int y) { return reinterpret_cast<const T*>(p.in + (size_t)y * p.in_pitch); }
template <typename T>
__device__ __forceinline__ T* out_row(const PixOp& p, int y) { return reinterpret_cast<T*>(p.out + (size_t)y * p.out_pitch); }

template <typename Ti>
__global__ __launch_bounds__(256) void k_depth_to_vbo(const PixOp p, const Intr K, const float scale)
{
    int u, v;
    pixel_xy(u, v);
    if (u >= p.w || v >= p.h) return;
    out_row<float4>(p, v)[u] = depth_vertex(K, scale * (float)in_row<Ti>(p, v)[u], u, v);
}

__global__ __launch_bounds__(256) void k_normals_from_vbo(const PixOp p)
{
    int u, v;
    pixel_xy(u, v);
    if (u >= p.w || v >= p.h) return;
    float4 N = make_float4(0.f, 0.f, 0.f, 0.f);
    if (u + 1 < p.w && v + 1 < p.h) N = vertex_normal(in_row<float4>(p, v)[u], in_row<float4>(p, v)[u + 1], in_row<float4>(p, v + 1)[u]);
    out_row<float4>(p, v)[u] = N;
}

struct VboNrmParams {
    const unsigned char* in;
    size_t in_pitch;
    unsigned char *vbo, *nrm;
    size_t vpitch, npitch;
    int w, h;
    Intr K;
    float scale;
    unsigned char* tex;
    size_t tpitch;
    float* bmax;
    unsigned bw8;
};
__device__ __forceinline__ float4 vertex_of(const VboNrmParams& p, int u, int v)
{
    return depth_vertex(p.K, p.scale * reinterpret_cast<const float*>(p.in + (size_t)v * p.in_pitch)[u], u, v);
}
__global__ __launch_bounds__(256) void k_vbo_normals_f32(const VboNrmParams p)
{
    __shared__ float s_max[PIX_H][8];
    int u, v, lane, wv;
    pixel_xy(u, v, lane, wv);
    float d = -__builtin_inff();
    if (u < p.w && v < p.h) {
        const float4 Vc = vertex_of(p, u, v);
        reinterpret_cast<float4*>(p.vbo + (size_t)v * p.vpitch)[u] = Vc;
        float4 N = make_float4(0.f, 0.f, 0.f, 0.f);
        if (u + 1 < p.w && v + 1 < p.h) N = vertex_normal(Vc, vertex_of(p, u + 1, v), vertex_of(p, u, v + 1));
        reinterpret_cast<float4*>(p.nrm + (size_t)v * p.npitch)[u] = N;
        if (p.tex) {
            d = reinterpret_cast<const float*>(p.in + (size_t)v * p.in_pitch)[u];
            texel_put(p.tex, p.tpitch, u, v, N, d);
        }
    }
    if (p.tex) texel_block_max(p.bmax, p.bw8, lane, wv, d, s_max);
}

template <typename Ti>
__global__ __launch_bounds__(256) void k_scale_bias(const PixOp p, const float s, const float offset)
{
    int x, y;
    pixel_xy(x, y);
    if (x >= p.w || y >= p.h) return;
    out_row<float>(p, y)[x] = scale_bias((float)in_row<Ti>(p, y)[x], s, offset);
}

__global__ __launch_bounds__(256) void k_box_half_ignore_invalid_f32(const PixOp p)
{
    int x, y;
    pixel_xy(x, y);
    if (x >= p.w || y >= p.h) return;
    const float2 t = *reinterpret_cast<const float2*>(in_row<float>(p, 2 * y) + 2 * x);
    const float2 b = *reinterpret_cast<const float2*>(in_row<float>(p, 2 * y + 1) + 2 * x);
    out_row<float>(p, y)[x] = box_half(t.x, t.y, b.x, b.y);
}

__global__ __launch_bounds__(256) void k_disp2depth(const PixOp p, float fu, float baseline, float min_disp)
{
    int x, y;
    pixel_xy(x, y);
    if (x >= p.w || y >= p.h) return;
    const float d = in_row<float>(p, y)[x];
    out_row<float>(p, y)[x] = d >= min_disp ? fu * baseline / d : __builtin_nanf("");
}

template <typename Ti>
__global__ __launch_bounds__(256) void k_filter_bad_kinect(const PixOp p)
{
    int x, y;
    pixel_xy(x, y);
    if (x >= p.w || y >= p.h) return;
    const float z_mm = (float)in_row<Ti>(p, y)[x];
    out_row<float>(p, y)[x] = z_mm >= 200 ? z_mm : __builtin_nanf("");
}

struct ColourVboParams {
    const unsigned char* vbo;
    size_t vpitch;
    const unsigned char* rgb;
    size_t rpitch;
    int rw, rh;
    unsigned char* out;
    size_t opitch;
    int w, h;
    Pose KT;
};

__global__ __launch_bounds__(256) void k_colour_vbo(const ColourVboParams p)
{
    int u, v;
    pixel_xy(u, v);
    if (u >= p.w || v >= p.h) return;
    const float4 Pd = *(reinterpret_cast<const float4*>(p.vbo + (size_t)v * p.vpitch) + u);
    const float k0 = p.KT.m[0] * Pd.x + p.KT.m[1] * Pd.y + p.KT.m[2] * Pd.z + p.KT.m[3] * 1.0f;
    const float k1 = p.KT.m[4] * Pd.x + p.KT.m[5] * Pd.y + p.KT.m[6] * Pd.z + p.KT.m[7] * 1.0f;
    const float k2 = p.KT.m[8] * Pd.x + p.KT.m[9] * Pd.y + p.KT.m[10] * Pd.z + p.KT.m[11] * 1.0f;
    const float pu = k0 / k2, pv = k1 / k2;
    uchar4 id = make_uchar4(0, 0, 0, 0);
    if (1.0f <= pu && pu < ((float)p.rw - 1.0f) && 1.0f <= pv && pv < ((float)p.rh - 1.0f)) {
        const V3 c = rgb_bilinear(p.rgb, p.rpitch, pu, pv);
        id = make_uchar4((unsigned char)c.x, (unsigned char)c.y, (unsigned char)c.z, 255);
    }
    *(reinterpret_cast<uchar4*>(p.out + (size_t)v * p.opitch) + u) = id;
// ... 230 lines not shown
extern "C" int kfx_box_half_ignore_invalid_f32(const kfx_image* out, const kfx_image* in, kfx_stream stream)
{
    PixOp p;
    if (int e = pix_op(p, out, 4, in, 4, 2, 2, "BoxHalfIgnoreInvalid: output image", "BoxHalfIgnoreInvalid: input image (2x the output)")) return e;
    if (empty(p)) return 0;
    if (((uintptr_t)in->ptr | in->pitch) & 7) return set_error(KFX_E_ALIGN, "BoxHalfIgnoreInvalid: input not 8-byte aligned");
    hipLaunchKernelGGL(k_box_half_ignore_invalid_f32, pixel_grid(p.w, p.h), dim3(256), 0, (hipStream_t)stream, p);
    return check_launch("kfx_box_half_ignore_invalid_f32");
}

extern "C" int kfx_disp2depth(const kfx_image* in, const kfx_image* out, float fu, float baseline, float min_disp, kfx_stream stream)
{
    PixOp p;
    if (int e = pix_op(p, out, 4, in, 4, 1, 1, "Disp2Depth: output image", "Disp2Depth: input image")) return e;
    if (empty(p)) return 0;
    hipLaunchKernelGGL(k_disp2depth, pixel_grid(p.w, p.h), dim3(256), 0, (hipStream_t)stream, p, fu, baseline, min_disp);
    return check_launch("kfx_disp2depth");
}

template <typename Ti>
static int filter_bad_kinect_launch(const kfx_image* out, const kfx_image* in, const char* name, kfx_stream stream)
{
    PixOp p;
    if (int e = pix_op(p, out, 4, in, sizeof(Ti), 1, 1, "FilterBadKinectData: output image", "FilterBadKinectData: input image")) return e;
    if (empty(p)) return 0;
    hipLaunchKernelGGL(k_filter_bad_kinect<Ti>, pixel_grid(p.w, p.h), dim3(256), 0, (hipStream_t)stream, p);
    return check_launch(name);
}
extern "C" int kfx_filter_bad_kinect_f32(const kfx_image* out, const kfx_image* in, kfx_stream stream)
{
    return filter_bad_kinect_launch<float>(out, in, "kfx_filter_bad_kinect_f32", stream);
}
extern "C" int kfx_filter_bad_kinect_u16(const kfx_image* out, const kfx_image* in, kfx_stream stream)
{
    return filter_bad_kinect_launch<unsigned short>(out, in, "kfx_filter_bad_kinect_u16", stream);
}

extern "C" int kfx_colour_vbo(const kfx_image* id, const kfx_image* vbo, const kfx_image* rgb, const float KT_cd[12], kfx_stream stream)
{
    if (int e = check_image(id, 4, 0, 0, "ColourVbo: output image")) return e;
    if (int e = check_image(vbo, 16, cover_w(id), cover_h(id), "ColourVbo: vbo image")) return e;
    if (int e = check_image(rgb, 3, 0, 0, "ColourVbo: rgb image")) return e;
    if (!KT_cd) return set_error(KFX_E_NULL, "ColourVbo: null transform");
    if (id->w == 0 || id->h == 0) return 0;
    ColourVboParams p;
    p.vbo = (const unsigned char*)vbo->ptr; p.vpitch = vbo->pitch;
    p.rgb = (const unsigned char*)rgb->ptr; p.rpitch = rgb->pitch; p.rw = (int)rgb->w; p.rh = (int)rgb->h;
    p.out = (unsigned char*)id->ptr; p.opitch = id->pitch; p.w = (int)id->w; p.h = (int)id->h;
    for (int i = 0; i < 12; ++i) p.KT.m[i] = KT_cd[i];
    hipLaunchKernelGGL(k_colour_vbo, pixel_grid(p.w, p.h), dim3(256), 0, (hipStream_t)stream, p);
    return check_launch("kfx_colour_vbo");
}

template <typename Tg>
static int guided_launch(const kfx_image* out, const kfx_image* in, const kfx_image* guide, float gs, float gr, float gc, unsigned size,
                         kfx_stream stream)
{
    if (int e = check_image(out, 4, 0, 0, "BilateralFilter(guided): output image")) return e;
    if (int e = check_image(in, 4, cover_w(out), cover_h(out), "BilateralFilter(guided): input image")) return e;
    if (int e = check_image(guide, sizeof(Tg), cover_w(out), cover_h(out), "BilateralFilter(guided): guide image")) return e;
    if (out->w == 0 || out->h == 0) return 0;
    if (size > 64) return set_error(KFX_E_RANGE, "BilateralFilter(guided): window too large");
    GuidedParams g;
    g.b = bil_params(out, in, gs, gr, size, 0.f, 0);
    g.guide = (const unsigned char*)guide->ptr;
    g.gpitch = guide->pitch;
    g.gw = (int)guide->w;
    g.gh = (int)guide->h;
    g.gc = gc;
    hipLaunchKernelGGL(k_bilateral_guided<Tg>, pixel_grid(g.b.w, g.b.h), dim3(256), 0, (hipStream_t)stream, g);
    return check_launch("kfx_bilateral_guided");
}
extern "C" int kfx_bilateral_guided_f32(const kfx_image* out, const kfx_image* in, const kfx_image* guide, float gs, float gr, float gc,
                                        unsigned size, kfx_stream stream)
{
    return guided_launch<float>(out, in, guide, gs, gr, gc, size, stream);
}
extern "C" int kfx_bilateral_guided_u8(const kfx_image* out, const kfx_image* in, const kfx_image* guide, float gs, float gr, float gc,
                                       unsigned size, kfx_stream stream)
{
    return guided_launch<unsigned char>(out, in, guide, gs, gr, gc, size, stream);
}

namespace kfx {
int depth_to_vbo_normals_texels(const kfx_image* vbo, const kfx_image* nrm, const kfx_image* depth, const float K[4], float scale,
                                const kfx_image* texels, kfx_stream stream);
}
extern "C" int kfx_depth_to_vbo_normals_f32(const kfx_image* vbo, const kfx_image* nrm, const kfx_image* depth, const float K[4], float scale,
                                            kfx_stream stream)
{
    return kfx::depth_to_vbo_normals_texels(vbo, nrm, depth, K, scale, nullptr, stream);
}
int kfx::depth_to_vbo_normals_texels(const kfx_image* vbo, const kfx_image* nrm, const kfx_image* depth, const float K[4], float scale,
                                     const kfx_image* texels, kfx_stream stream)
{
    if (int e = check_image(vbo, 16, 0, 0, "DepthToVbo+Normals: vbo image")) return e;
    if (int e = check_image(nrm, 16, 0, 0, "DepthToVbo+Normals: normal image")) return e;
    if (int e = check_image(depth, 4, cover_w(vbo), cover_h(vbo), "DepthToVbo+Normals: depth image")) return e;
    if (!K) return set_error(KFX_E_NULL, "DepthToVbo+Normals: null intrinsics");
    if (vbo->w == 0 || vbo->h == 0) return 0;
    if (nrm->w != vbo->w || nrm->h != vbo->h) return set_error(KFX_E_SHAPE, "DepthToVbo+Normals: vbo and normals differ in size");
    const TexLayout tl = tex_layout(vbo->w, vbo->h);
    if (texels && (!texels->ptr || texels->w != vbo->w || texels->h != vbo->h || texels->pitch != tl.tpitch || ((uintptr_t)texels->ptr & 15)))
        return set_error(KFX_E_SHAPE, "DepthToVbo+Normals: texel image");
    VboNrmParams p{(const unsigned char*)depth->ptr, depth->pitch, (unsigned char*)vbo->ptr, (unsigned char*)nrm->ptr, vbo->pitch, nrm->pitch,
                   (int)vbo->w, (int)vbo->h, Intr{K[0], K[1], K[2], K[3]}, scale, texels ? (unsigned char*)texels->ptr : nullptr, texels ? tl.tpitch : 0,
                   texels ? reinterpret_cast<float*>((unsigned char*)texels->ptr + tl.bmax_off) : nullptr, tl.bw8};
    hipLaunchKernelGGL(k_vbo_normals_f32, pixel_grid(p.w, p.h), dim3(256), 0, (hipStream_t)stream, p);
    return check_launch("kfx_depth_to_vbo_normals_f32");
}

struct PyrParams {
    const unsigned char* d0;
    size_t d0_pitch;
    unsigned char* d[4];
    size_t dpitch[4];
    unsigned char *vbo[4], *nrm[4];
    size_t vpitch[4], npitch[4];
    int w[4], h[4];
    Intr K[4];
    int levels;
    float scale;
};
__global__ __launch_bounds__(256) void k_depth_pyramid_vbo_normals(const PyrParams p)
{
    constexpr int E0 = 40, E1 = 20, E2 = 10, E3 = 5;
    __shared__ float s0[E0 * E0], s1[E1 * E1], s2[E2 * E2], s3[E3 * E3];
    const int tid = threadIdx.x;
    {
        const int x0 = blockIdx.x * 32, y0 = blockIdx.y * 32;
        for (int t = tid; t < E0 * E0; t += 256) {
            const int ly = t / E0, lx = t - ly * E0, x = x0 + lx, y = y0 + ly;
            s0[t] = (x < p.w[0] && y < p.h[0]) ? reinterpret_cast<const float*>(p.d0 + (size_t)y * p.d0_pitch)[x] : 0.f;
        }
    }
    __syncthreads();
    float* const sl[4] = {s0, s1, s2, s3};
    const int ext[4] = {E0, E1, E2, E3};
#pragma unroll
    for (int l = 1; l < 4; ++l) {
        if (l < p.levels) {
            const int E = ext[l], Ef = ext[l - 1], S = 32 >> l;
            const int x0 = blockIdx.x * S, y0 = blockIdx.y * S;
            const float* f = sl[l - 1];
            for (int t = tid; t < E * E; t += 256) {
                const int ly = t / E, lx = t - ly * E;
                const float m = box_half(f[(2 * ly) * Ef + 2 * lx], f[(2 * ly) * Ef + 2 * lx + 1], f[(2 * ly + 1) * Ef + 2 * lx], f[(2 * ly + 1) * Ef + 2 * lx + 1]);
                sl[l][t] = m;
                const int x = x0 + lx, y = y0 + ly;
                if (lx < S && ly < S && x < p.w[l] && y < p.h[l]) reinterpret_cast<float*>(p.d[l] + (size_t)y * p.dpitch[l])[x] = m;
            }
        }
        __syncthreads();
    }
#pragma unroll
    for (int l = 0; l < 4; ++l) {
        if (l >= p.levels) break;
        const int E = ext[l], S = 32 >> l, w = p.w[l], h = p.h[l];
        const int x0 = blockIdx.x * S, y0 = blockIdx.y * S;
        const float* d = sl[l];
        const Intr K = p.K[l];
        for (int t = tid; t < S * S; t += 256) {
            const int ly = t / S, lx = t - ly * S, u = x0 + lx, v = y0 + ly;
            if (u >= w || v >= h) continue;
            const float4 Vc = depth_vertex(K, p.scale * d[ly * E + lx], u, v);
            reinterpret_cast<float4*>(p.vbo[l] + (size_t)v * p.vpitch[l])[u] = Vc;
            float4 N = make_float4(0.f, 0.f, 0.f, 0.f);
            if (u + 1 < w && v + 1 < h)
                N = vertex_normal(Vc, depth_vertex(K, p.scale * d[ly * E + lx + 1], u + 1, v), depth_vertex(K, p.scale * d[(ly + 1) * E + lx], u, v + 1));
            reinterpret_cast<float4*>(p.nrm[l] + (size_t)v * p.npitch[l])[u] = N;
        }
    }
}

extern "C" int kfx_depth_pyramid_vbo_normals_f32(const kfx_image* depth, const kfx_image* vbo, const kfx_image* nrm, const float* K, int levels,
                                                 float scale, kfx_stream stream)
{
    if (!depth || !vbo || !nrm || !K) return set_error(KFX_E_NULL, "DepthPyramidVboNormals: null argument");
    if (levels < 1 || levels > 4) return set_error(KFX_E_RANGE, "DepthPyramidVboNormals: 1 to 4 levels");
    PyrParams p;
    p.levels = levels;
    p.scale = scale;
    for (int l = 0; l < 4; ++l) {
        p.d[l] = p.vbo[l] = p.nrm[l] = nullptr;
        p.dpitch[l] = p.vpitch[l] = p.npitch[l] = 0;
        p.w[l] = p.h[l] = 0;
        p.K[l] = Intr{1.f, 1.f, 0.f, 0.f};
    }
    for (int l = 0; l < levels; ++l) {
        if (int e = check_image(&depth[l], 4, 0, 0, "DepthPyramidVboNormals: depth image")) return e;
        if (int e = check_image(&vbo[l], 16, 0, 0, "DepthPyramidVboNormals: vbo image")) return e;
// ... 54 lines not shown
```

### kangaroo_amd/csrc/slab_frame.hip

```cpp
#include <cmath>
#include <cstdlib>
#include <new>

#include "kfx_device.h"
#include "frame_host.h"
#include "../../include/kfx_slab.h"
#include "slab_internal.h"

namespace {
constexpr int EV = 5;
constexpr int OPEN_SLOTS = 8;
constexpr int PIPE_MAX = KFX_SLAB_PIPE_MAX;
struct PendingFinal { long long frame; int set, os; };
}

struct kfx_slab_frame {
    kfx_slab_frame_config cfg;
    kfx_comm* comm;
    long long frames;
    void* exact;     size_t exact_bytes;
    void* strips;    size_t strips_bytes;
    void* keys;      size_t keys_bytes;
    void* bcast;     size_t bcast_bytes;
    int* h_open;
// ... 293 lines not shown
    if (merge >= 0) c.merge = merge;
    if (inputs >= 0) c.inputs = inputs;
    if (overlap >= 0) c.overlap = overlap ? 1 : 0;
    if (tiles >= 0) c.tiles = tiles;
    if (int e = check_policies(c, f->comm->world)) return e;
    FirstError note;
    note(flush_pending(f));
    note(hip_status(hipDeviceSynchronize(), "kfx_slab_frame_configure"));
    settle(f);
    const int o = check_open(f, true);
    if (!note.status) note(ensure_scratch(f, c));
    if (int e = ranks_agree(f, note.status)) return e;
    f->cfg = c;
    f->pipe = pipe_of(c, f->comm->world);
    return o;
}

extern "C" int kfx_slab_frame_reset(kfx_slab_frame* f, kfx_stream stream)
{
    if (!f) return set_error(KFX_E_NULL, "kfx_slab_frame_reset: null frame");
    if (int e = kfx_sdf_reset(&f->cfg.local, __builtin_nanf(""), stream)) return e;
    return f->color ? kfx_color_reset(&f->cvol, stream) : 0;
}

extern "C" int kfx_slab_frame_set_color(kfx_slab_frame* f, const kfx_volume* color_local, const kfx_image* rgb, const float Kimg[4], const float* T_cd)
{
    if (!f) return set_error(KFX_E_NULL, "kfx_slab_frame_set_color: null frame");
    if (!color_local) {
        f->color = 0;
        return 0;
    }
    if (!rgb || !rgb->ptr || !Kimg) return set_error(KFX_E_NULL, "kfx_slab_frame_set_color: null argument");
    if (int e = check_volume(color_local, 4, 1, VOLUME_MAX_DIM, "kfx_slab_frame_set_color")) return e;
    if (int e = check_color_slab(&f->cfg.local, color_local, "kfx_slab_frame_set_color")) return e;
    if (int e = check_image(rgb, 3, 4, 4, "kfx_slab_frame_set_color: rgb image (4 x 4 or larger)")) return e;
    f->cvol = *color_local;
    f->rgb = *rgb;
    for (int i = 0; i < 4; ++i) f->Kimg[i] = Kimg[i];
    static const float identity[12] = {1, 0, 0, 0, 0, 1, 0, 0, 0, 0, 1, 0};
    for (int i = 0; i < 12; ++i) f->T_cd[i] = T_cd ? T_cd[i] : identity[i];
    f->color = 1;
    return 0;
}

extern "C" int kfx_slab_frame_step(kfx_slab_frame* f, const kfx_image* raw, const float T_wc[12], const float* T_cw, unsigned parts, kfx_stream stream)
{
    if (!f || !T_wc) return set_error(KFX_E_NULL, "kfx_slab_frame_step: null argument");
    if (parts == 0) parts = KFX_FRAME_PREPROCESS | KFX_FRAME_FUSE | KFX_FRAME_RAYCAST;
    const kfx_slab_frame_config& c = f->cfg;
    const kfx_slab_layout& L = c.layout;
    kfx_comm* comm = f->comm;
    const int world = comm->world, rank = comm->rank;
    const kfx_image* src = raw ? raw : &c.raw;
    float inv[12];
    if (!T_cw) {
        se3_inverse(T_wc, inv);
        T_cw = inv;
    }
    if ((parts & KFX_FRAME_RAYCAST) &&
        ((c.raycast == KFX_SLAB_RAYCAST_EXACT && !f->exact) ||
         (c.raycast == KFX_SLAB_RAYCAST_COMPOSITE && world > 1 && !(c.merge == KFX_SLAB_MERGE_DIRECT ? f->strips : f->keys))))
        return set_error(KFX_E_NULL, "kfx_slab_frame_step: no scratch for the configured raycast (a failed kfx_slab_frame_configure)");
    if ((parts & KFX_FRAME_PREPROCESS) && c.inputs == KFX_SLAB_INPUTS_BROADCAST && world > 1 && !f->bcast)
        return set_error(KFX_E_NULL, "kfx_slab_frame_step: no scratch for the input broadcast (a failed kfx_slab_frame_configure)");
    const hipStream_t s = (hipStream_t)stream;
    FirstError note;
    ring_begin(f->ring, f->frames, f->timing);
    const auto record = [&](int k, hipStream_t on) {
        if (ring_record(f->ring, f->frames, k, on) != hipSuccess) note(set_error(KFX_E_RANGE, "kfx_slab_frame_step: hipEventRecord"));
    };
    if (f->merge_pending && (parts & KFX_FRAME_RAYCAST)) {
        note(hip_status(hipStreamWaitEvent(s, f->merged, 0), "kfx_slab_frame_step: hipStreamWaitEvent"));
        f->merge_pending = 0;
    }
    note(check_open(f, false));

    record(0, s);
    const kfx_image* tex = ((parts & KFX_FRAME_PREPROCESS) && (parts & KFX_FRAME_FUSE) && f->texels.ptr &&
                            !(c.inputs == KFX_SLAB_INPUTS_BROADCAST && world > 1 && rank != 0)) ? &f->texels : nullptr;
    if (parts & KFX_FRAME_PREPROCESS) {
        const bool bcast = c.inputs == KFX_SLAB_INPUTS_BROADCAST && world > 1;
        if (!bcast || rank == 0) {
            note(kfx_bilateral_f32(&c.filtered, src, c.bilateral_gs, c.bilateral_gr, c.bilateral_size, c.bilateral_minval, 1, stream));
            note(kfx::depth_to_vbo_normals_texels(&c.vbo, &c.normals, &c.filtered, c.K, 1.0f, tex, stream));
        }
        if (bcast) note(kfx_slab_broadcast_inputs(&c.filtered, &c.normals, f->bcast, 0, comm, stream));
    }
    record(1, s);
    if (parts & KFX_FRAME_FUSE) {
        const bool own_only = c.halo == KFX_SLAB_HALO_EXCHANGE && world > 1;
        const size_t first = own_only ? L.z0 : L.s0, count = own_only ? L.z1 - L.z0 : L.s1 - L.s0;
        const auto planes = [&](kfx_volume v) { v.ptr = (unsigned char*)v.ptr + (first - L.s0) * v.img_pitch; v.d = count; return v; };
        const kfx_volume v = planes(c.local);
        const kfx_slab sl = {L.full_d, first, L.full_zmin, L.full_zmax};
        if (f->color) {
            const kfx_volume cv = planes(f->cvol);
            float T_iw[12];
            for (int i = 0; i < 3; ++i)
                for (int j = 0; j < 4; ++j) {
                    float a = 0.f;
                    for (int k = 0; k < 3; ++k) a += f->T_cd[i * 4 + k] * T_cw[k * 4 + j];
                    T_iw[i * 4 + j] = j == 3 ? a + f->T_cd[i * 4 + 3] : a;
                }
            note(kfx_sdf_fuse_color_slab(&v, &cv, &sl, &c.filtered, &c.normals, T_cw, c.K, &f->rgb, T_iw, f->Kimg, c.trunc_dist, c.max_w, c.mincostheta,
                                         KFX_FUSE_SLAB_EXTENT, stream));
        } else {
            note(kfx::sdf_fuse_slab_texels(&v, &sl, &c.filtered, &c.normals, tex, T_cw, c.K, c.trunc_dist, c.max_w, c.mincostheta, KFX_FUSE_SLAB_EXTENT, stream));
        }
        if (own_only) note(kfx_slab_exchange_halos(&c.local, &L, comm, stream));
        if (own_only && f->color) note(kfx_slab_exchange_halos(&f->cvol, &L, comm, stream));
    }
    record(2, s);
    if (parts & KFX_FRAME_RAYCAST) {
        if (c.raycast == KFX_SLAB_RAYCAST_EXACT) {
            const int os = (int)(f->frames % OPEN_SLOTS);
            if (take_open_slot(f, os, true)) note(open_rays_error());
            int steps = 0;
            const int tiles = c.tiles ? c.tiles : 4;
            if (f->pipe > 0) {
                const int set = (int)(f->frames % f->pipe);
                if (f->fin_inflight[set]) {
                    note(hip_status(hipStreamWaitEvent(s, f->fin_done[set], 0), "kfx_slab_frame_step: hipStreamWaitEvent"));
                    f->fin_inflight[set] = 0;
                }
                kfx::TiledScratch t;
                kfx::tiled_layout(t, f->exact, c.ray_img.w, c.ray_img.h, tiles, world);
                note(kfx::exact_tiled_march(t, f->fin[set], &c.local, &L, T_wc, c.K, c.near, c.far, c.trunc_dist, 1, (int)c.ray_img.w, (int)c.ray_img.h, comm,
                                            stream, &steps, f->color ? &f->cvol : nullptr));
                f->last_steps = steps;
                record(3, s);
                note(hip_status(hipEventRecord(f->marched_ev[set], s), "kfx_slab_frame_step: hipEventRecord"));
                f->pending[f->n_pending++] = PendingFinal{f->frames, set, os};
                const int lag = (f->side_comm.flags & KFX_COMM_HOST_BLOCKING) ? f->pipe - 1 : 0;
                while (f->n_pending > lag) note(finalise_oldest(f));
            } else {
                note(kfx::exact_tiled(&c.ray_depth, &c.ray_norm, &c.ray_img, f->exact, &c.local, f->color ? &f->cvol : nullptr, &L, T_wc, c.K, c.near, c.far,
                                      c.trunc_dist, 1, tiles, comm, stream, f->h_open + os, &steps));
                f->last_steps = steps;
                if (hipEventRecord(f->open_done[os], s) == hipSuccess) f->open_frame[os] = f->frames;
                else (void)hipGetLastError();
                record(3, s);
            }
        } else {
            if (f->color) note(kfx_raycast_sdf_color(&c.ray_depth, &c.ray_norm, &c.ray_img, &c.local, &f->cvol, T_wc, c.K, c.near, c.far, c.trunc_dist, 1, stream));
            else note(kfx_raycast_sdf(&c.ray_depth, &c.ray_norm, &c.ray_img, &c.local, T_wc, c.K, c.near, c.far, c.trunc_dist, 1, stream));
            record(3, s);
            if (world > 1) {
                hipStream_t ms = s;
                if (c.overlap) {
                    note(hip_status(hipEventRecord(f->marched, s), "kfx_slab_frame_step: hipEventRecord"));
                    note(hip_status(hipStreamWaitEvent(f->side, f->marched, 0), "kfx_slab_frame_step: hipStreamWaitEvent"));
                    ms = f->side;
                }
                if (c.merge == KFX_SLAB_MERGE_DIRECT) {
                    note(kfx_slab_composite_direct(&c.ray_depth, &c.ray_norm, &c.ray_img, f->strips, comm, (kfx_stream)ms));
                } else {
                    long long* key = static_cast<long long*>(f->keys);
                    float* payload = reinterpret_cast<float*>(key + c.ray_img.w * c.ray_img.h + 2);
                    payload = reinterpret_cast<float*>(((uintptr_t)payload + 15) & ~(uintptr_t)15);
                    note(kfx_slab_composite(&c.ray_depth, &c.ray_norm, &c.ray_img, key, payload, comm, (kfx_stream)ms));
                }
                record(4, ms);
                if (c.overlap) {
                    note(hip_status(hipEventRecord(f->merged, f->side), "kfx_slab_frame_step: hipEventRecord"));
                    f->merge_pending = 1;
                }
            }
// ... 32 lines not shown
```

Measured before the change: 2641.

## Precompute per-brick fuse plan inside the normals kernel and read it in fuse

Adds a per-brick plan buffer (tile rect, zmin, bad/miss/inside flags). Extra workgroups appended to the vbo/normals preprocessing kernel compute it, and the fuse kernel loads the entry from constant memory instead of projecting brick corners and doing wave reductions at block start. The per-brick setup latency moves off the fuse critical path into a kernel that was underutilised. The cost is an extra buffer, extra workgroups in preprocessing, and a plan that only matches the pose for the current frame.

```diff
diff --git a/include/kfx_debug.h b/include/kfx_debug.h
--- a/include/kfx_debug.h
+++ b/include/kfx_debug.h
@@ -25,6 +25,8 @@
 
 int kfx_debug_fuse_keep(const kfx_sdf_summary* s, int out[3], unsigned char* kept, int n_rows);
 
+int kfx_debug_fuse_plan(int dims_out[3], unsigned* plan_out, unsigned* inwave_out);
+
 #ifdef __cplusplus
 }
 #endif
diff --git a/kangaroo_amd/csrc/debug.hip b/kangaroo_amd/csrc/debug.hip
--- a/kangaroo_amd/csrc/debug.hip
+++ b/kangaroo_amd/csrc/debug.hip
@@ -1,4 +1,5 @@
 #include "kfx_device.h"
+#include "fuse_plan.h"
 #include "sampling.h"
 #include "../../include/kfx_debug.h"
 
@@ -319,3 +320,54 @@
         kept[r] = (r >= s->keep_row0 && r < s->keep_row0 + s->keep_rows && keep_row(r, s->keep_stride)) ? 1 : 0;
     return 0;
 }
+
+namespace kfx {
+__global__ __launch_bounds__(64) void k_debug_brick_setup(const FuseParams p, uint4* __restrict__ out)
+{
+    const int lane = threadIdx.x;
+    const int zbeg = blockIdx.z * FUSE_ZC, zend = min(zbeg + FUSE_ZC, p.Z);
+    const BrickCorner k = brick_corner<true>(p, lane & 7, (int)blockIdx.x * TB_X, (int)blockIdx.y * TB_Y, TB_X, TB_Y, slice_z(p, (lane & 4) ? zend - 1 : zbeg));
+    const FMin fmin2;
+    const FMax fmax2;
+    const auto uni = [](float x) { return __uint_as_float((unsigned)__builtin_amdgcn_readfirstlane((int)__float_as_uint(x))); };
+    const float umin = uni(wave8_combine(k.pu, fmin2)), umax = uni(wave8_combine(k.pu, fmax2));
+    const float vmin = uni(wave8_combine(k.pv, fmin2)), vmax = uni(wave8_combine(k.pv, fmax2));
+    const float zmin = uni(wave8_combine(k.Pc.z, fmin2));
+    const bool any_bad = __ballot(k.bad) != 0ull;
+    bool miss = false, inside = false;
+    TileRect tile = {0, 0, 0, 0};
+    if (!any_bad) {
+        miss = misses_band(umin, umax, vmin, vmax, p.dwb, p.dhb);
+        if (!miss) {
+            tile = tile_rect(umin, umax, vmin, vmax, p.depth.w, p.depth.h);
+            inside = inside_band(umin, umax, vmin, vmax, p.dwb, p.dhb);
+        }
+    }
+    if (lane == 0)
+        out[((size_t)blockIdx.z * gridDim.y + blockIdx.y) * gridDim.x + blockIdx.x] =
+            plan_pack(tile, zmin, (any_bad ? PLAN_BAD : 0u) | (miss ? PLAN_MISS : 0u) | (inside ? PLAN_INSIDE : 0u));
+}
+}
+
+extern "C" int kfx_debug_fuse_plan(int dims_out[3], unsigned* plan_out, unsigned* inwave_out)
+{
+    if (!dims_out) return set_error(KFX_E_NULL, "kfx_debug_fuse_plan: null argument");
+    dims_out[0] = dims_out[1] = dims_out[2] = 0;
+    const FusePlanUsed* u = fuse_plan_last();
+    if (!u || !u->entries) return 1;
+    dims_out[0] = u->g.nbx; dims_out[1] = u->g.nby; dims_out[2] = u->g.nbz;
+    const size_t bytes = plan_bytes(u->g);
+    if (int e = hip_status(hipDeviceSynchronize(), "kfx_debug_fuse_plan: hipDeviceSynchronize")) return e;
+    if (plan_out)
+        if (int e = hip_status(hipMemcpy(plan_out, u->entries, bytes, hipMemcpyDeviceToHost), "kfx_debug_fuse_plan: hipMemcpy")) return e;
+    if (inwave_out) {
+        void* buf = nullptr;
+        if (int e = hip_status(hipMalloc(&buf, bytes), "kfx_debug_fuse_plan: hipMalloc")) return e;
+        hipLaunchKernelGGL(k_debug_brick_setup, dim3(u->g.nbx, u->g.nby, u->g.nbz), dim3(64), 0, nullptr, u->p, (uint4*)buf);
+        int e = check_launch("kfx_debug_fuse_plan");
+        if (!e) e = hip_status(hipMemcpy(inwave_out, buf, bytes, hipMemcpyDeviceToHost), "kfx_debug_fuse_plan: hipMemcpy");
+        (void)hipFree(buf);
+        if (e) return e;
+    }
+    return 0;
+}
diff --git a/kangaroo_amd/csrc/frame.hip b/kangaroo_amd/csrc/frame.hip
--- a/kangaroo_amd/csrc/frame.hip
+++ b/kangaroo_amd/csrc/frame.hip
@@ -15,6 +15,7 @@
     kfx::EventRing ring;
     unsigned mask;
     kfx_image texels;
+    kfx::PlanRef plan;
     kfx_depth_input* input;
 };
 
@@ -36,8 +37,10 @@
     f->mask = KFX_FRAME_EVENTS_ALL;
     f->input = nullptr;
     f->texels = texel_image_alloc(cfg->filtered.w, cfg->filtered.h);
+    f->plan = plan_alloc(cfg->vol.w, cfg->vol.h, cfg->vol.d);
     if (int e = ring_create(f->ring, 4, cfg->timing_slots, -1, "kfx_frame_create")) {
         texel_image_free(f->texels);
+        plan_free(f->plan);
         delete f;
         return e;
     }
@@ -51,6 +54,7 @@
     if (f->summary) kfx_sdf_summary_destroy(f->summary);
     ring_destroy(f->ring);
     texel_image_free(f->texels);
+    plan_free(f->plan);
     delete f;
     return 0;
 }
@@ -126,11 +130,13 @@
     if (!e && (parts & KFX_FRAME_PREPROCESS)) {
         if (sensor) e = depth_input_consume(sensor, &c.filtered, &c.raw, c.bilateral_gs, c.bilateral_gr, c.bilateral_size, c.bilateral_minval, stream);
         else e = kfx_bilateral_f32(&c.filtered, src, c.bilateral_gs, c.bilateral_gr, c.bilateral_size, c.bilateral_minval, 1, stream);
-        if (!e) e = depth_to_vbo_normals_texels(&c.vbo, &c.normals, &c.filtered, c.K, 1.0f, tex, stream);
+        PlanJob job;
+        const bool planned = tex && fuse_plan_prepare(&job, &f->plan, &c.vol, &c.filtered, &c.normals, T_cw, c.K, c.trunc_dist, c.max_w, c.mincostheta, c.fuse_flags);
+        if (!e) e = depth_to_vbo_normals_texels(&c.vbo, &c.normals, &c.filtered, c.K, 1.0f, tex, planned ? &job : nullptr, stream);
     }
     record(1);
     if (!e && (parts & KFX_FRAME_FUSE))
-        e = sdf_fuse_texels(&c.vol, f->track ? f->summary : nullptr, &c.filtered, &c.normals, tex, T_cw, c.K, c.trunc_dist, c.max_w, c.mincostheta, c.fuse_flags, stream);
+        e = sdf_fuse_texels(&c.vol, f->track ? f->summary : nullptr, &c.filtered, &c.normals, tex, tex ? &f->plan : nullptr, T_cw, c.K, c.trunc_dist, c.max_w, c.mincostheta, c.fuse_flags, stream);
     record(2);
     if (!e && (parts & KFX_FRAME_RAYCAST)) {
         if (f->track) e = kfx_raycast_sdf_tracked(&c.ray_depth, &c.ray_norm, &c.ray_img, &c.vol, f->summary, T_wc, c.K, c.near, c.far, c.trunc_dist, 1, stream);
diff --git a/kangaroo_amd/csrc/frame_host.h b/kangaroo_amd/csrc/frame_host.h
--- a/kangaroo_amd/csrc/frame_host.h
+++ b/kangaroo_amd/csrc/frame_host.h
@@ -2,7 +2,10 @@
 
 #include <new>
 
+#include <cstring>
+
 #include "kfx_device.h"
+#include "fuse_plan.h"
 #include "host_args.h"
 
 namespace kfx {
@@ -39,6 +42,21 @@
     if (tl.tpitch < (1u << 24) && hipMalloc(&buf, tl.bytes) == hipSuccess) return kfx_image{tl.tpitch, buf, w, h};
     (void)hipGetLastError();
     return kfx_image{0, nullptr, 0, 0};
+}
+inline PlanRef plan_alloc(size_t w, size_t h, size_t d)
+{
+    PlanRef r;
+    memset(&r, 0, sizeof(r));
+    const size_t bytes = plan_bytes(plan_grid((int)w, (int)h, (int)d));
+    void* buf = nullptr;
+    if (bytes && hipMalloc(&buf, bytes) == hipSuccess) { r.entries = (uint4*)buf; r.bytes = bytes; }
+    else (void)hipGetLastError();
+    return r;
+}
+inline void plan_free(PlanRef& r)
+{
+    if (r.entries) { (void)hipFree(r.entries); (void)hipGetLastError(); }
+    memset(&r, 0, sizeof(r));
 }
 inline void texel_image_free(kfx_image& t)
 {
diff --git a/kangaroo_amd/csrc/fuse.hip b/kangaroo_amd/csrc/fuse.hip
--- a/kangaroo_amd/csrc/fuse.hip
+++ b/kangaroo_amd/csrc/fuse.hip
@@ -9,6 +9,7 @@
 #include <type_traits>
 
 #include "kfx_device.h"
+#include "fuse_plan.h"
 #include "../../include/kfx_slab_color.h"
 #include "host_args.h"
 
@@ -18,72 +19,11 @@
 
 namespace kfx {
 
-constexpr int FUSE_ZC = 16;
 constexpr int FUSE_ROWS = 4;
-constexpr int TB_X = 64, TB_Y = 8;
-
-struct FuseParams {
-    unsigned char* vptr;
-    size_t vpitch, vimg_pitch;
-    int X, Y, Z;
-    int zoff;
-    float w1, h1, d1;
-    V3 bmin, size;
-    Pose T;
-    Intr K;
-    ImgView depth;
-    ImgView norm;
-    float dwb, dhb;
-    float trunc, max_w, mincos;
-    unsigned dpitch, npitch;
-    int exact_shared;
-    int z_rev, keep_stride, keep_row0;
-    float4* sum_R;
-    int sum_nbx, sum_nby;
-    int sum_bx0, sum_by0, sum_bz0;
-    int sum_w, sum_h, sum_d;
-    float sum_lo_ok, sum_hi_ok;
-    int* sum_dirty;
-    int zoff_local;
-    int xcd_swizzle;
-    int fuse_cull;
-    const unsigned char* tex;
-    unsigned tpitch;
-    const float* bmax;
-    unsigned bw8;
-    float inv_w1, inv_h1;
-    int pos_div;
-};
-
-__device__ __forceinline__ float voxel_pos(float bmin, float size, int i, float n1, float inv_n1, int pos_div)
-{
-    const float a = size * (float)i;
-    return bmin + (pos_div ? div_uniform(a, n1, inv_n1) : a / n1);
-}
-
-__device__ __forceinline__ float slice_z(const FuseParams& p, int z) { return p.bmin.z + p.size.z * (float)(z + p.zoff) / p.d1; }
 
 __device__ __forceinline__ int xcd_rotated_brick(const FuseParams& p, int bzi)
 {
     return p.xcd_swizzle ? (int)((blockIdx.x + (bzi >> (p.xcd_swizzle - 1))) % gridDim.x) : (int)blockIdx.x;
-}
-
-struct TileRect {
-    int x0, y0, w, h;
-    __device__ __forceinline__ bool fits(int cap) const { return w > 1 && h > 1 && w * h <= cap; }
-};
-__device__ __forceinline__ TileRect tile_rect(float lo_u, float hi_u, float lo_v, float hi_v, int img_w, int img_h)
-{
-    const float fx0 = fmaxf(floorf(lo_u) - 1.f, 0.f), fx1 = fminf(floorf(hi_u) + 2.f, (float)(img_w - 1));
-    const float fy0 = fmaxf(floorf(lo_v) - 1.f, 0.f), fy1 = fminf(floorf(hi_v) + 2.f, (float)(img_h - 1));
-    TileRect r;
-    r.x0 = (int)fx0; r.y0 = (int)fy0;
-    r.w = (int)fx1 - r.x0 + 1; r.h = (int)fy1 - r.y0 + 1;
-    return r;
-}
-__device__ __forceinline__ bool misses_band(float lo_u, float hi_u, float lo_v, float hi_v, float wb, float hb)
-{
-    return hi_u < 2.0f || !(lo_u < wb) || hi_v < 2.0f || !(lo_v < hb);
 }
 
 __device__ __forceinline__ float far_depth(float dmax) { return dmax + fabsf(dmax) * 1e-5f; }
@@ -113,44 +53,6 @@
 typedef float v4f __attribute__((ext_vector_type(4)));
 
 __device__ __forceinline__ float lerp_f(float a, float b, float t) { return __builtin_fmaf(t, b - a, a); }
-
-template <bool FAST>
-struct CamXY {
-    float ax, ay, az;
-    __device__ __forceinline__ void init(const FuseParams& p, float px, float py)
-    {
-        if constexpr (FAST) {
-            ax = __builtin_fmaf(p.T.m[0], px, __builtin_fmaf(p.T.m[1], py, p.T.m[3]));
-            ay = __builtin_fmaf(p.T.m[4], px, __builtin_fmaf(p.T.m[5], py, p.T.m[7]));
-            az = __builtin_fmaf(p.T.m[8], px, __builtin_fmaf(p.T.m[9], py, p.T.m[11]));
-        } else {
-            ax = p.T.m[0] * px + p.T.m[1] * py;
-            ay = p.T.m[4] * px + p.T.m[5] * py;
-            az = p.T.m[8] * px + p.T.m[9] * py;
-        }
-    }
-    __device__ __forceinline__ V3 at(const FuseParams& p, float pz) const
-    {
-        if constexpr (FAST)
-            return v3(__builtin_fmaf(p.T.m[2], pz, ax), __builtin_fmaf(p.T.m[6], pz, ay), __builtin_fmaf(p.T.m[10], pz, az));
-        else
-            return v3(ax + p.T.m[2] * pz + p.T.m[3], ay + p.T.m[6] * pz + p.T.m[7], az + p.T.m[10] * pz + p.T.m[11]);
-    }
-};
-
-template <bool FAST>
-__device__ __forceinline__ void project(const FuseParams& p, const V3 Pc, float& pu, float& pv, float& iz)
-{
-    if constexpr (FAST) {
-        iz = __builtin_amdgcn_rcpf(Pc.z);
-        pu = __builtin_fmaf(p.K.fu * Pc.x, iz, p.K.u0);
-        pv = __builtin_fmaf(p.K.fv * Pc.y, iz, p.K.v0);
-    } else {
-        iz = 0.f;
-        pu = p.K.u0 + p.K.fu * Pc.x / Pc.z;
-        pv = p.K.v0 + p.K.fv * Pc.y / Pc.z;
-    }
-}
 
 __device__ __forceinline__ bool in_bounds(const FuseParams& p, float pu, float pv)
 {
@@ -448,6 +350,24 @@
     const int zend = min(zbeg + ZC, p.Z);
     const int wz0 = zbeg + (wv / WY) * ZW, wz1 = min(wz0 + ZW, zend);
     const bool live = x0 < p.X && y < p.Y;
+    constexpr bool PLANNED = FAST && !DXT && CELL::BYTES == 8 && LX == 32 && WY == 4 && NW == 4 && ZC == FUSE_ZC;
+    typedef unsigned v4u __attribute__((ext_vector_type(4)));
+    v4u plan_e = {0u, 0u, 0u, 0u};
+    if constexpr (PLANNED) {
+        if (p.plan != nullptr) {
+            const size_t at = ((size_t)(p.plan_bz0 + bzi) * gridDim.y + blockIdx.y) * gridDim.x + (size_t)bxi;
+            plan_e = *(const __attribute__((address_space(4))) v4u*)(p.plan + at);
+        } else {
+            const int c = lane & 7;
+            const BrickCorner k = brick_corner<FAST>(p, c, bxi * LX * 2, (int)blockIdx.y * BY, LX * 2, BY, slice_z(p, (c & 4) ? zend - 1 : zbeg));
+            const FMin fmin2;
+            const FMax fmax2;
+            const uint4 e = plan_entry(wave8_combine(k.pu, fmin2), wave8_combine(k.pu, fmax2), wave8_combine(k.pv, fmin2), wave8_combine(k.pv, fmax2),
+                                       wave8_combine(k.Pc.z, fmin2), __ballot(k.bad) != 0ull, p);
+            plan_e = v4u{(unsigned)__builtin_amdgcn_readfirstlane((int)e.x), (unsigned)__builtin_amdgcn_readfirstlane((int)e.y),
+                         (unsigned)__builtin_amdgcn_readfirstlane((int)e.z), (unsigned)__builtin_amdgcn_readfirstlane((int)e.w)};
+        }
+    }
     if (tid < ZC) {
         const float pz = slice_z(p, zbeg + tid);
         s_pz[tid] = pz;
@@ -460,41 +380,42 @@
 #pragma unroll
     for (int v = 0; v < 2; ++v) cam[v].init(p, voxel_pos(p.bmin.x, p.size.x, x0 + v, p.w1, p.inv_w1, p.pos_div), py);
 
-    float umin, umax, vmin, vmax, zmin, cmax = 0.f;
-    bool any_bad;
-    {
+    float umin = 0.f, umax = 0.f, vmin = 0.f, vmax = 0.f, zmin = 0.f, cmax = 0.f;
+    bool any_bad = false, miss = false, inside = false;
+    TileRect tile = {0, 0, 0, 0};
+    if constexpr (!PLANNED) {
         const int c = lane & 7;
-        const int xb0 = bxi * LX * 2, yb0 = (int)blockIdx.y * BY;
-        const int xc = (c & 1) ? min(xb0 + LX * 2, p.X) - 1 : xb0;
-        const int yc = (c & 2) ? min(yb0 + BY, p.Y) - 1 : yb0;
-        const float pzc = s_pz[(c & 4) ? (zend - 1 - zbeg) : 0];
-        CamXY<FAST> cc;
-        cc.init(p, voxel_pos(p.bmin.x, p.size.x, xc, p.w1, p.inv_w1, p.pos_div), voxel_pos(p.bmin.y, p.size.y, yc, p.h1, p.inv_h1, p.pos_div));
-        const V3 Pc = cc.at(p, pzc);
-        float pu, pv, iz;
-        project<FAST>(p, Pc, pu, pv, iz);
-        const bool bad = !(Pc.z > 0.f) || !(fabsf(pu) < 1e9f) || !(fabsf(pv) < 1e9f);
+        const BrickCorner k = brick_corner<FAST>(p, c, bxi * LX * 2, (int)blockIdx.y * BY, LX * 2, BY, s_pz[(c & 4) ? (zend - 1 - zbeg) : 0]);
         const FMin fmin2;
         const FMax fmax2;
         const auto uni = [](float x) { return __uint_as_float((unsigned)__builtin_amdgcn_readfirstlane((int)__float_as_uint(x))); };
-        umin = uni(wave8_combine(pu, fmin2)); umax = uni(wave8_combine(pu, fmax2));
-        vmin = uni(wave8_combine(pv, fmin2)); vmax = uni(wave8_combine(pv, fmax2));
-        zmin = uni(wave8_combine(Pc.z, fmin2));
-        if constexpr (!FAST) cmax = uni(wave8_combine(fmaxf(fmaxf(fabsf(Pc.x), fabsf(Pc.y)), Pc.z), fmax2));
-        any_bad = __ballot(bad) != 0ull;
+        umin = uni(wave8_combine(k.pu, fmin2)); umax = uni(wave8_combine(k.pu, fmax2));
+        vmin = uni(wave8_combine(k.pv, fmin2)); vmax = uni(wave8_combine(k.pv, fmax2));
+        zmin = uni(wave8_combine(k.Pc.z, fmin2));
+        if constexpr (!FAST) cmax = uni(wave8_combine(fmaxf(fmaxf(fabsf(k.Pc.x), fabsf(k.Pc.y)), k.Pc.z), fmax2));
+        any_bad = __ballot(k.bad) != 0ull;
+    }
+    if constexpr (PLANNED) {
+        tile.x0 = (int)(plan_e.x & 0xFFFFu); tile.y0 = (int)(plan_e.x >> 16);
+        tile.w = (int)(plan_e.y & 0xFFFFu); tile.h = (int)(plan_e.y >> 16);
+        zmin = __uint_as_float(plan_e.z);
+        any_bad = (plan_e.w & PLAN_BAD) != 0u; miss = (plan_e.w & PLAN_MISS) != 0u; inside = (plan_e.w & PLAN_INSIDE) != 0u;
     }
 
     bool use_tile = false;
-    TileRect tile = {0, 0, 0, 0};
     if (!any_bad) {
-        if (misses_band(umin, umax, vmin, vmax, p.dwb, p.dhb)) return;
-        tile = tile_rect(umin, umax, vmin, vmax, p.depth.w, p.depth.h);
+        if constexpr (PLANNED) {
+            if (miss) return;
+        } else {
+            if (misses_band(umin, umax, vmin, vmax, p.dwb, p.dhb)) return;
+            tile = tile_rect(umin, umax, vmin, vmax, p.depth.w, p.depth.h);
+        }
         use_tile = tile.fits(cap_px);
         if constexpr (DXT) use_tile = use_tile && p.exact_shared && zmin >= 0x1p-20f && cmax <= 0x1p20f;
     }
     const int tx0 = tile.x0, ty0 = tile.y0, tw = tile.w, th = tile.h;
     const bool whole = !TRACK || ((bxi + 1) * LX * 2 <= p.X && ((int)blockIdx.y + 1) * BY <= p.Y);
-    const bool interior = __builtin_amdgcn_readfirstlane((int)(use_tile && whole && umin >= 2.01f && umax < p.dwb - 0.01f && vmin >= 2.01f && vmax < p.dhb - 0.01f)) != 0;
+    const bool interior = __builtin_amdgcn_readfirstlane((int)(use_tile && whole && (PLANNED ? inside : inside_band(umin, umax, vmin, vmax, p.dwb, p.dhb)))) != 0;
     float dmax = -__builtin_inff();
     constexpr bool DMA = KFX_FUSE_STAGE_DMA && !DXT;
     if constexpr (DMA) {
@@ -784,7 +705,8 @@
             }
         }
         if (use_tile) {
-            const int cxmax = PARK ? in_vgpr(tw - 2) : tw - 2, cymax = PARK ? in_vgpr(th - 2) : th - 2, tx0v = PARK ? in_vgpr(tx0) : tx0,
+            constexpr bool PARK_LIM = PARK && !PLANNED;
+            const int cxmax = PARK_LIM ? in_vgpr(tw - 2) : tw - 2, cymax = PARK_LIM ? in_vgpr(th - 2) : th - 2, tx0v = PARK ? in_vgpr(tx0) : tx0,
                       ty0v = PARK ? in_vgpr(ty0) : ty0;
             auto tiled_loop = [&](auto interior_c) {
             constexpr bool INTERIOR = decltype(interior_c)::value;
@@ -1359,9 +1281,13 @@
 using namespace kfx;
 
 __global__ __launch_bounds__(256) void k_pack_texels(const ImgView depth, const ImgView norm, unsigned char* __restrict__ tex, const size_t tpitch,
-                                                     float* __restrict__ bmax, const unsigned bw8)
+                                                     float* __restrict__ bmax, const unsigned bw8, const int rows, const PlanJob job)
 {
     __shared__ float s_max[PIX_H][8];
+    if ((int)blockIdx.y >= rows) {
+        plan_write(job.p, job.out, job.g, ((int)blockIdx.y - rows) * (int)gridDim.x + (int)blockIdx.x);
+        return;
+    }
     int u, v, lane, wv;
     pixel_xy(u, v, lane, wv);
     float d = -__builtin_inff();
@@ -1549,6 +1475,36 @@
     return TilePlan{small_brick, 3328, 0};
 }
 
+static int fuse_plan_env()
+{
+    static const int plan = env_int("KFX_FUSE_PLAN", 1);
+    return plan;
+}
+static PlanTag plan_tag(const FuseParams& p)
+{
+    PlanTag t;
+    memset(&t, 0, sizeof(t));
+    t.X = p.X; t.Y = p.Y; t.Z = p.Z; t.zoff = p.zoff;
+    t.w1 = p.w1; t.h1 = p.h1; t.d1 = p.d1; t.inv_w1 = p.inv_w1; t.inv_h1 = p.inv_h1;
+    t.pos_div = p.pos_div;
+    t.bmin = p.bmin; t.size = p.size;
+    t.T = p.T; t.K = p.K;
+    t.img_w = p.depth.w; t.img_h = p.depth.h;
+    t.bx = TB_X; t.by = TB_Y; t.bz = FUSE_ZC;
+    return t;
+}
+static bool plan_possible(const FuseParams& p, bool fast, size_t cell_bytes, const kfx_slab* slab)
+{
+    return fuse_plan_env() && fast && cell_bytes == 8 && !slab && p.depth.w < PLAN_MAX_IMG && p.depth.h < PLAN_MAX_IMG &&
+           p.X > 0 && p.Y > 0 && p.Z > 0;
+}
+static FusePlanUsed& last_plan()
+{
+    thread_local FusePlanUsed used = {};
+    return used;
+}
+const FusePlanUsed* kfx::fuse_plan_last() { return &last_plan(); }
+
 static int fuse_tiled_env()
 {
     static const int tiled = env_int("KFX_FUSE_TILED", 1);
@@ -1644,10 +1600,12 @@
 template <typename CELL>
 static int fuse_launch(const kfx_volume* vol, const kfx_image* depth, const kfx_image* norm, const float T_cw[12],
                        const float K[4], float trunc_dist, float max_w, float mincostheta, unsigned flags, kfx_stream stream,
-                       const kfx_slab* slab = nullptr, kfx_sdf_summary* summary = nullptr, const kfx_image* texels = nullptr)
+                       const kfx_slab* slab = nullptr, kfx_sdf_summary* summary = nullptr, const kfx_image* texels = nullptr,
+                       const PlanRef* plan = nullptr)
 {
     FuseParams p;
     bool small_images = false;
+    last_plan().entries = nullptr;
     if (int e = fuse_params(p, &small_images, vol, depth, norm, T_cw, K, trunc_dist, max_w, mincostheta, flags, CELL::BYTES, slab)) return e;
     if (summary && summary->cell_bytes != CELL::BYTES)
         return set_error(KFX_E_SHAPE, "SdfFuse(tracked): the summary was created for the other cell type (kfx_sdf_summary_create / _create_h)");
@@ -1701,15 +1659,28 @@
         for (int ri = 0; ri < n_ranges; ++ri) any_plain = any_plain || !ranges[ri].plan.dxt;
         if (KFX_FUSE_STAGE_DMA && any_plain) {
             const TexLayout tl = tex_layout(depth->w, depth->h);
+            bool want_plan = false;
+            if (plan_possible(p, fast, CELL::BYTES, slab))
+                for (int ri = 0; ri < n_ranges; ++ri) want_plan = want_plan || !ranges[ri].plan.small_brick;
+            const PlanTag tag = plan_tag(p);
             if (texels && texels->ptr && texels->w == depth->w && texels->h == depth->h && texels->pitch == tl.tpitch && !((uintptr_t)texels->ptr & 15)) {
                 p.tex = (const unsigned char*)texels->ptr;
+                if (want_plan && plan && plan->valid && plan->entries && memcmp(&plan->tag, &tag, sizeof(tag)) == 0) p.plan = plan->entries;
             } else {
-                void* buf = tex_scratch(tl.bytes, s);
+                const PlanGrid g = plan_grid(p.X, p.Y, p.Z);
+                const size_t plan_off = (tl.bytes + 15) & ~(size_t)15;
+                void* buf = tex_scratch(plan_off + (want_plan ? plan_bytes(g) : 0), s);
                 if (!buf) return set_error((int)hipErrorOutOfMemory, "SdfFuse: no device memory for the packed texel image");
-                hipLaunchKernelGGL(k_pack_texels, pixel_grid((int)depth->w, (int)depth->h), dim3(256), 0, s, p.depth, p.norm,
-                                   (unsigned char*)buf, tl.tpitch, reinterpret_cast<float*>((unsigned char*)buf + tl.bmax_off), tl.bw8);
+                dim3 grid = pixel_grid((int)depth->w, (int)depth->h);
+                const int rows = (int)grid.y;
+                PlanJob job = {p, g, want_plan ? reinterpret_cast<uint4*>((unsigned char*)buf + plan_off) : nullptr};
+                if (want_plan) grid.y += (unsigned)plan_rows(g, (int)grid.x);
+                hipLaunchKernelGGL(k_pack_texels, grid, dim3(256), 0, s, p.depth, p.norm,
+                                   (unsigned char*)buf, tl.tpitch, reinterpret_cast<float*>((unsigned char*)buf + tl.bmax_off), tl.bw8, rows, job);
                 p.tex = (const unsigned char*)buf;
-            }
+                p.plan = job.out;
+            }
+            if (p.plan) last_plan() = FusePlanUsed{p.plan, plan_grid(p.X, p.Y, p.Z), p};
             p.tpitch = (unsigned)tl.tpitch;
             p.bmax = reinterpret_cast<const float*>(p.tex + tl.bmax_off);
             p.bw8 = tl.bw8;
@@ -1722,6 +1693,8 @@
             FuseParams q = z_range(p, rg.z0, rg.z1);
             q.z_rev = rev;
             q.keep_stride = keep_stride; q.keep_row0 = p.sum_by0;
+            q.plan = plan.small_brick ? nullptr : p.plan;
+            q.plan_bz0 = rg.z0 / FUSE_ZC;
             const size_t lds = (size_t)cap_px * sizeof(float4) * (plan.dxt ? 2 : 1);
             const int zu = zu_env ? zu_env : (fast ? (cap_px > 2560 ? 4 : 2) : 1);
             const bool nw8 = fast && nw8_from > 0 && cap_px > nw8_from;
@@ -1744,9 +1717,26 @@
 }
 
 int kfx::sdf_fuse_texels(const kfx_volume* vol, kfx_sdf_summary* summary, const kfx_image* depth, const kfx_image* norm, const kfx_image* texels,
-                         const float T_cw[12], const float K[4], float trunc_dist, float max_w, float mincostheta, unsigned flags, kfx_stream stream)
-{
-    return fuse_launch<CellF32>(vol, depth, norm, T_cw, K, trunc_dist, max_w, mincostheta, flags, stream, nullptr, summary, texels);
+                         const PlanRef* plan, const float T_cw[12], const float K[4], float trunc_dist, float max_w, float mincostheta, unsigned flags,
+                         kfx_stream stream)
+{
+    return fuse_launch<CellF32>(vol, depth, norm, T_cw, K, trunc_dist, max_w, mincostheta, flags, stream, nullptr, summary, texels, plan);
+}
+
+int kfx::fuse_plan_prepare(PlanJob* job, PlanRef* ref, const kfx_volume* vol, const kfx_image* depth, const kfx_image* norm, const float T_cw[12],
+                           const float K[4], float trunc_dist, float max_w, float mincostheta, unsigned flags)
+{
+    ref->valid = 0;
+    bool small_images = false;
+    if (!ref->entries || !vol || !vol->ptr || !depth || !norm || !T_cw || !K) return 0;
+    if (fuse_params(job->p, &small_images, vol, depth, norm, T_cw, K, trunc_dist, max_w, mincostheta, flags, CellF32::BYTES, nullptr)) return 0;
+    if (!plan_possible(job->p, math_mode() == KFX_MATH_FAST, CellF32::BYTES, nullptr) || !small_images || !fuse_tiled_env()) return 0;
+    job->g = plan_grid(job->p.X, job->p.Y, job->p.Z);
+    if (plan_bytes(job->g) > ref->bytes) return 0;
+    job->out = ref->entries;
+    ref->tag = plan_tag(job->p);
+    ref->valid = 1;
+    return 1;
 }
 
 int kfx::sdf_fuse_slab_texels(const kfx_volume* vol, const kfx_slab* slab, const kfx_image* depth, const kfx_image* norm, const kfx_image* texels,
diff --git a/kangaroo_amd/csrc/fuse_plan.h b/kangaroo_amd/csrc/fuse_plan.h
--- /dev/null
+++ b/kangaroo_amd/csrc/fuse_plan.h
@@ -0,0 +1,207 @@
+#pragma once
+
+#include "kfx_device.h"
+
+namespace kfx {
+
+constexpr int FUSE_ZC = 16;
+constexpr int TB_X = 64, TB_Y = 8;
+
+struct FuseParams {
+    unsigned char* vptr;
+    size_t vpitch, vimg_pitch;
+    int X, Y, Z;
+    int zoff;
+    float w1, h1, d1;
+    V3 bmin, size;
+    Pose T;
+    Intr K;
+    ImgView depth;
+    ImgView norm;
+    float dwb, dhb;
+    float trunc, max_w, mincos;
+    unsigned dpitch, npitch;
+    int exact_shared;
+    int z_rev, keep_stride, keep_row0;
+    float4* sum_R;
+    int sum_nbx, sum_nby;
+    int sum_bx0, sum_by0, sum_bz0;
+    int sum_w, sum_h, sum_d;
+    float sum_lo_ok, sum_hi_ok;
+    int* sum_dirty;
+    int zoff_local;
+    int xcd_swizzle;
+    int fuse_cull;
+    const unsigned char* tex;
+    unsigned tpitch;
+    const float* bmax;
+    unsigned bw8;
+    float inv_w1, inv_h1;
+    int pos_div;
+    const uint4* plan;
+    int plan_bz0;
+};
+
+__device__ __forceinline__ float voxel_pos(float bmin, float size, int i, float n1, float inv_n1, int pos_div)
+{
+    const float a = size * (float)i;
+    return bmin + (pos_div ? div_uniform(a, n1, inv_n1) : a / n1);
+}
+
+__device__ __forceinline__ float slice_z(const FuseParams& p, int z) { return p.bmin.z + p.size.z * (float)(z + p.zoff) / p.d1; }
+
+struct TileRect {
+    int x0, y0, w, h;
+    __device__ __forceinline__ bool fits(int cap) const { return w > 1 && h > 1 && w * h <= cap; }
+};
+__device__ __forceinline__ TileRect tile_rect(float lo_u, float hi_u, float lo_v, float hi_v, int img_w, int img_h)
+{
+    const float fx0 = fmaxf(floorf(lo_u) - 1.f, 0.f), fx1 = fminf(floorf(hi_u) + 2.f, (float)(img_w - 1));
+    const float fy0 = fmaxf(floorf(lo_v) - 1.f, 0.f), fy1 = fminf(floorf(hi_v) + 2.f, (float)(img_h - 1));
+    TileRect r;
+    r.x0 = (int)fx0; r.y0 = (int)fy0;
+    r.w = (int)fx1 - r.x0 + 1; r.h = (int)fy1 - r.y0 + 1;
+    return r;
+}
+__device__ __forceinline__ bool misses_band(float lo_u, float hi_u, float lo_v, float hi_v, float wb, float hb)
+{
+    return hi_u < 2.0f || !(lo_u < wb) || hi_v < 2.0f || !(lo_v < hb);
+}
+__device__ __forceinline__ bool inside_band(float lo_u, float hi_u, float lo_v, float hi_v, float wb, float hb)
+{
+    return lo_u >= 2.01f && hi_u < wb - 0.01f && lo_v >= 2.01f && hi_v < hb - 0.01f;
+}
+
+template <bool FAST>
+struct CamXY {
+    float ax, ay, az;
+    __device__ __forceinline__ void init(const FuseParams& p, float px, float py)
+    {
+        if constexpr (FAST) {
+            ax = __builtin_fmaf(p.T.m[0], px, __builtin_fmaf(p.T.m[1], py, p.T.m[3]));
+            ay = __builtin_fmaf(p.T.m[4], px, __builtin_fmaf(p.T.m[5], py, p.T.m[7]));
+            az = __builtin_fmaf(p.T.m[8], px, __builtin_fmaf(p.T.m[9], py, p.T.m[11]));
+        } else {
+            ax = p.T.m[0] * px + p.T.m[1] * py;
+            ay = p.T.m[4] * px + p.T.m[5] * py;
+            az = p.T.m[8] * px + p.T.m[9] * py;
+        }
+    }
+    __device__ __forceinline__ V3 at(const FuseParams& p, float pz) const
+    {
+        if constexpr (FAST)
+            return v3(__builtin_fmaf(p.T.m[2], pz, ax), __builtin_fmaf(p.T.m[6], pz, ay), __builtin_fmaf(p.T.m[10], pz, az));
+        else
+            return v3(ax + p.T.m[2] * pz + p.T.m[3], ay + p.T.m[6] * pz + p.T.m[7], az + p.T.m[10] * pz + p.T.m[11]);
+    }
+};
+
+template <bool FAST>
+__device__ __forceinline__ void project(const FuseParams& p, const V3 Pc, float& pu, float& pv, float& iz)
+{
+    if constexpr (FAST) {
+        iz = __builtin_amdgcn_rcpf(Pc.z);
+        pu = __builtin_fmaf(p.K.fu * Pc.x, iz, p.K.u0);
+        pv = __builtin_fmaf(p.K.fv * Pc.y, iz, p.K.v0);
+    } else {
+        iz = 0.f;
+        pu = p.K.u0 + p.K.fu * Pc.x / Pc.z;
+        pv = p.K.v0 + p.K.fv * Pc.y / Pc.z;
+    }
+}
+
+struct BrickCorner { V3 Pc; float pu, pv; bool bad; };
+template <bool FAST>
+__device__ __forceinline__ BrickCorner brick_corner(const FuseParams& p, int c, int xb0, int yb0, int bx, int by, float pzc)
+{
+    const int xc = (c & 1) ? min(xb0 + bx, p.X) - 1 : xb0;
+    const int yc = (c & 2) ? min(yb0 + by, p.Y) - 1 : yb0;
+    CamXY<FAST> cc;
+    cc.init(p, voxel_pos(p.bmin.x, p.size.x, xc, p.w1, p.inv_w1, p.pos_div), voxel_pos(p.bmin.y, p.size.y, yc, p.h1, p.inv_h1, p.pos_div));
+    BrickCorner r;
+    r.Pc = cc.at(p, pzc);
+    float iz;
+    project<FAST>(p, r.Pc, r.pu, r.pv, iz);
+    r.bad = !(r.Pc.z > 0.f) || !(fabsf(r.pu) < 1e9f) || !(fabsf(r.pv) < 1e9f);
+    return r;
+}
+
+constexpr unsigned PLAN_BAD = 1u, PLAN_MISS = 2u, PLAN_INSIDE = 4u;
+constexpr int PLAN_MAX_IMG = 32768;
+
+struct PlanGrid { int nbx, nby, nbz; };
+inline PlanGrid plan_grid(int X, int Y, int Z) { return PlanGrid{ceil_div(X, TB_X), ceil_div(Y, TB_Y), ceil_div(Z, FUSE_ZC)}; }
+inline size_t plan_bytes(const PlanGrid& g) { return (size_t)g.nbx * g.nby * g.nbz * sizeof(uint4); }
+
+__device__ __forceinline__ uint4 plan_pack(const TileRect& t, float zmin, unsigned flags)
+{
+    return make_uint4((unsigned)t.x0 | ((unsigned)t.y0 << 16), (unsigned)t.w | ((unsigned)t.h << 16), __float_as_uint(zmin), flags);
+}
+
+__device__ __forceinline__ uint4 plan_entry(float umin, float umax, float vmin, float vmax, float zmin, bool any_bad, const FuseParams& p)
+{
+    unsigned flags = 0u;
+    TileRect t = {0, 0, 0, 0};
+    if (any_bad) flags = PLAN_BAD;
+    else if (misses_band(umin, umax, vmin, vmax, p.dwb, p.dhb)) flags = PLAN_MISS;
+    else {
+        t = tile_rect(umin, umax, vmin, vmax, p.depth.w, p.depth.h);
+        if (inside_band(umin, umax, vmin, vmax, p.dwb, p.dhb)) flags = PLAN_INSIDE;
+    }
+    return plan_pack(t, zmin, flags);
+}
+
+struct PlanTag {
+    int X, Y, Z, zoff;
+    float w1, h1, d1, inv_w1, inv_h1;
+    int pos_div;
+    V3 bmin, size;
+    Pose T;
+    Intr K;
+    int img_w, img_h;
+    int bx, by, bz;
+};
+
+struct PlanRef {
+    uint4* entries;
+    size_t bytes;
+    PlanTag tag;
+    int valid;
+};
+
+constexpr int PLAN_BRICKS_PER_WG = 32;
+inline int plan_workgroups(const PlanGrid& g) { return ceil_div(g.nbx * g.nby * g.nbz, PLAN_BRICKS_PER_WG); }
+inline int plan_rows(const PlanGrid& g, int grid_x) { return ceil_div(plan_workgroups(g), grid_x); }
+
+struct PlanJob {
+    FuseParams p;
+    PlanGrid g;
+    uint4* out;
+};
+
+struct FusePlanUsed {
+    const uint4* entries;
+    PlanGrid g;
+    FuseParams p;
+};
+const FusePlanUsed* fuse_plan_last();
+
+__device__ __forceinline__ void plan_write(const FuseParams& p, uint4* __restrict__ plan, const PlanGrid g, int wg)
+{
+    const int n = g.nbx * g.nby * g.nbz;
+    if (wg * PLAN_BRICKS_PER_WG >= n) return;
+    const int b = min(wg * PLAN_BRICKS_PER_WG + (int)(threadIdx.x >> 3), n - 1);
+    const int bxi = b % g.nbx, byi = (b / g.nbx) % g.nby, bzi = b / (g.nbx * g.nby);
+    const int zbeg = bzi * FUSE_ZC, zend = min(zbeg + FUSE_ZC, p.Z);
+    const int c = (int)(threadIdx.x & 7);
+    const BrickCorner k = brick_corner<true>(p, c, bxi * TB_X, byi * TB_Y, TB_X, TB_Y, slice_z(p, (c & 4) ? zend - 1 : zbeg));
+    const FMin fmin2;
+    const FMax fmax2;
+    const float umin = wave8_combine(k.pu, fmin2), umax = wave8_combine(k.pu, fmax2);
+    const float vmin = wave8_combine(k.pv, fmin2), vmax = wave8_combine(k.pv, fmax2);
+    const float zmin = wave8_combine(k.Pc.z, fmin2);
+    const bool any_bad = ((__ballot(k.bad) >> (threadIdx.x & 56u)) & 0xFFull) != 0ull;
+    if ((threadIdx.x & 7) == 0) plan[b] = plan_entry(umin, umax, vmin, vmax, zmin, any_bad, p);
+}
+
+}
diff --git a/kangaroo_amd/csrc/kfx_device.h b/kangaroo_amd/csrc/kfx_device.h
--- a/kangaroo_amd/csrc/kfx_device.h
+++ b/kangaroo_amd/csrc/kfx_device.h
@@ -339,10 +339,15 @@
 int check_launch(const char* what);
 int hip_status(hipError_t e, const char* what);
 int math_mode();
+struct PlanJob;
+struct PlanRef;
+int fuse_plan_prepare(PlanJob* job, PlanRef* ref, const kfx_volume* vol, const kfx_image* depth, const kfx_image* norm, const float T_cw[12],
+                      const float K[4], float trunc_dist, float max_w, float mincostheta, unsigned flags);
 int depth_to_vbo_normals_texels(const kfx_image* vbo, const kfx_image* nrm, const kfx_image* depth, const float K[4], float scale,
-                                const kfx_image* texels, kfx_stream stream);
+                                const kfx_image* texels, const PlanJob* job, kfx_stream stream);
 int sdf_fuse_slab_texels(const kfx_volume* vol, const kfx_slab* slab, const kfx_image* depth, const kfx_image* norm, const kfx_image* texels,
                          const float T_cw[12], const float K[4], float trunc_dist, float max_w, float mincostheta, unsigned flags, kfx_stream stream);
 int sdf_fuse_texels(const kfx_volume* vol, kfx_sdf_summary* summary, const kfx_image* depth, const kfx_image* norm, const kfx_image* texels,
-                    const float T_cw[12], const float K[4], float trunc_dist, float max_w, float mincostheta, unsigned flags, kfx_stream stream);
-}
+                    const PlanRef* plan, const float T_cw[12], const float K[4], float trunc_dist, float max_w, float mincostheta, unsigned flags,
+                    kfx_stream stream);
+}
diff --git a/kangaroo_amd/csrc/preprocess.hip b/kangaroo_amd/csrc/preprocess.hip
--- a/kangaroo_amd/csrc/preprocess.hip
+++ b/kangaroo_amd/csrc/preprocess.hip
@@ -1,5 +1,6 @@
 
 #include "kfx_device.h"
+#include "fuse_plan.h"
 #include "host_args.h"
 #include "sensor_host.h"
 
@@ -245,14 +246,19 @@
     size_t tpitch;
     float* bmax;
     unsigned bw8;
+    int rows;
 };
 __device__ __forceinline__ float4 vertex_of(const VboNrmParams& p, int u, int v)
 {
     return depth_vertex(p.K, p.scale * reinterpret_cast<const float*>(p.in + (size_t)v * p.in_pitch)[u], u, v);
 }
-__global__ __launch_bounds__(256) void k_vbo_normals_f32(const VboNrmParams p)
+__global__ __launch_bounds__(256) void k_vbo_normals_f32(const VboNrmParams p, const PlanJob job)
 {
     __shared__ float s_max[PIX_H][8];
+    if ((int)blockIdx.y >= p.rows) {
+        plan_write(job.p, job.out, job.g, ((int)blockIdx.y - p.rows) * (int)gridDim.x + (int)blockIdx.x);
+        return;
+    }
     int u, v, lane, wv;
     pixel_xy(u, v, lane, wv);
     float d = -__builtin_inff();
@@ -649,17 +655,13 @@
     return guided_launch<unsigned char>(out, in, guide, gs, gr, gc, size, stream);
 }
 
-namespace kfx {
-int depth_to_vbo_normals_texels(const kfx_image* vbo, const kfx_image* nrm, const kfx_image* depth, const float K[4], float scale,
-                                const kfx_image* texels, kfx_stream stream);
-}
 extern "C" int kfx_depth_to_vbo_normals_f32(const kfx_image* vbo, const kfx_image* nrm, const kfx_image* depth, const float K[4], float scale,
                                             kfx_stream stream)
 {
-    return kfx::depth_to_vbo_normals_texels(vbo, nrm, depth, K, scale, nullptr, stream);
+    return kfx::depth_to_vbo_normals_texels(vbo, nrm, depth, K, scale, nullptr, nullptr, stream);
 }
 int kfx::depth_to_vbo_normals_texels(const kfx_image* vbo, const kfx_image* nrm, const kfx_image* depth, const float K[4], float scale,
-                                     const kfx_image* texels, kfx_stream stream)
+                                     const kfx_image* texels, const PlanJob* job, kfx_stream stream)
 {
     if (int e = check_image(vbo, 16, 0, 0, "DepthToVbo+Normals: vbo image")) return e;
     if (int e = check_image(nrm, 16, 0, 0, "DepthToVbo+Normals: normal image")) return e;
@@ -672,8 +674,14 @@
         return set_error(KFX_E_SHAPE, "DepthToVbo+Normals: texel image");
     VboNrmParams p{(const unsigned char*)depth->ptr, depth->pitch, (unsigned char*)vbo->ptr, (unsigned char*)nrm->ptr, vbo->pitch, nrm->pitch,
                    (int)vbo->w, (int)vbo->h, Intr{K[0], K[1], K[2], K[3]}, scale, texels ? (unsigned char*)texels->ptr : nullptr, texels ? tl.tpitch : 0,
-                   texels ? reinterpret_cast<float*>((unsigned char*)texels->ptr + tl.bmax_off) : nullptr, tl.bw8};
-    hipLaunchKernelGGL(k_vbo_normals_f32, pixel_grid(p.w, p.h), dim3(256), 0, (hipStream_t)stream, p);
+                   texels ? reinterpret_cast<float*>((unsigned char*)texels->ptr + tl.bmax_off) : nullptr, tl.bw8, 0};
+    dim3 grid = pixel_grid(p.w, p.h);
+    p.rows = (int)grid.y;
+    PlanJob none;
+    memset(&none, 0, sizeof(none));
+    if (job && job->out) grid.y += (unsigned)plan_rows(job->g, (int)grid.x);
+    else job = &none;
+    hipLaunchKernelGGL(k_vbo_normals_f32, grid, dim3(256), 0, (hipStream_t)stream, p, *job);
     return check_launch("kfx_depth_to_vbo_normals_f32");
 }
 
diff --git a/kangaroo_amd/csrc/slab_frame.hip b/kangaroo_amd/csrc/slab_frame.hip
--- a/kangaroo_amd/csrc/slab_frame.hip
+++ b/kangaroo_amd/csrc/slab_frame.hip
@@ -399,7 +399,7 @@
         const bool bcast = c.inputs == KFX_SLAB_INPUTS_BROADCAST && world > 1;
         if (!bcast || rank == 0) {
             note(kfx_bilateral_f32(&c.filtered, src, c.bilateral_gs, c.bilateral_gr, c.bilateral_size, c.bilateral_minval, 1, stream));
-            note(kfx::depth_to_vbo_normals_texels(&c.vbo, &c.normals, &c.filtered, c.K, 1.0f, tex, stream));
+            note(kfx::depth_to_vbo_normals_texels(&c.vbo, &c.normals, &c.filtered, c.K, 1.0f, tex, nullptr, stream));
         }
         if (bcast) note(kfx_slab_broadcast_inputs(&c.filtered, &c.normals, f->bcast, 0, comm, stream));
     }
```

Result: no change. 2657 (median of 6 runs) (+0.6%).
